# robertknight/ocrs

Hardware: AMD Instinct MI355X
Metric: pages/sec end-to-end (1024x1024) (higher is better)
Workload: dtype f32

## Files before the change

include/ocrs_amd.h:

```cpp
#ifndef OCRS_AMD_H
#define OCRS_AMD_H

#include <stddef.h>
#include <stdint.h>

#if defined(__GNUC__)
#define OCRS_API __attribute__((visibility("default")))
#else
#define OCRS_API
#endif

#ifdef __cplusplus
extern "C" {
#endif

typedef enum ocrs_status {
    OCRS_OK = 0,
    OCRS_ERR_INVALID_ARGUMENT = 1,
    OCRS_ERR_MODEL_NOT_LOADED = 2,
    OCRS_ERR_MODEL_DIMS = 3,
    OCRS_ERR_RUN_FAILED = 4,
    OCRS_ERR_WRONG_OUTPUT = 5,
    OCRS_ERR_IMAGE_SOURCE = 6,
    OCRS_ERR_DEVICE = 7,
    OCRS_ERR_IO = 8,
    OCRS_ERR_CAPACITY = 9
} ocrs_status;

OCRS_API const char* ocrs_last_error(void);

#define OCRS_ABI_VERSION 6u
OCRS_API uint32_t ocrs_abi_version(void);

OCRS_API void ocrs_buffer_free(void* p);

OCRS_API ocrs_status ocrs_device_count(int* n);
OCRS_API ocrs_status ocrs_set_device(int device);
OCRS_API ocrs_status ocrs_get_device(int* device);

OCRS_API ocrs_status ocrs_ctc_beam_search(const float* logp, int t, int c, uint32_t width, int impl, uint32_t** labels,
                                          uint32_t** positions, size_t* n);
OCRS_API ocrs_status ocrs_ctc_beam_search_scored(const float* logp, int t, int c, uint32_t width, int impl, uint32_t** labels,
                                                 uint32_t** positions, size_t* n, double* score, float** step_logp);

OCRS_API ocrs_status ocrs_gru_tile_plan(const int32_t* lengths_desc, size_t n_lines, int hidden, int32_t* n_clusters, int32_t* waves,
                                        int16_t* tiles);

OCRS_API ocrs_status ocrs_coalescer_selftest(int n_threads, int requests_per_thread, int max_active, int max_pages,
                                             long window_us, int fail_every, uint64_t out[5]);

OCRS_API ocrs_status ocrs_set_option(const char* name, long value);
OCRS_API ocrs_status ocrs_option_name(int index, const char** name);

OCRS_API ocrs_status ocrs_device_pool_stats(int device, uint64_t out[12]);
OCRS_API ocrs_status ocrs_device_pool_configure(int device, uint64_t device_cached_cap_bytes, uint64_t pinned_cached_cap_bytes);
OCRS_API ocrs_status ocrs_device_pool_trim(int device);

typedef enum { OCRS_ISOLATION_AUTO = 0, OCRS_ISOLATION_NONE = 1 } ocrs_isolation;
OCRS_API ocrs_status ocrs_device_set_isolation(int device, ocrs_isolation policy);
OCRS_API ocrs_status ocrs_device_isolation(int device, int out[3]);

typedef struct ocrs_model ocrs_model;

OCRS_API ocrs_status ocrs_model_load_file(const char* path, ocrs_model** out);
OCRS_API ocrs_status ocrs_model_load_bytes(const void* data, size_t len, ocrs_model** out);
OCRS_API ocrs_status ocrs_model_load_file_on_device(const char* path, int device, ocrs_model** out);
OCRS_API ocrs_status ocrs_model_load_bytes_on_device(const void* data, size_t len, int device, ocrs_model** out);
OCRS_API ocrs_status ocrs_model_device(const ocrs_model* m, int* device);

typedef int (*ocrs_model_run_fn)(void* user, const float* input, const int64_t in_shape[4], float** output,
                                 int64_t out_shape[4], int* out_ndim);
OCRS_API ocrs_status ocrs_model_from_callback(const int64_t input_shape[4],
                                     ocrs_model_run_fn run, void* user, ocrs_model** out);

OCRS_API ocrs_status ocrs_model_input_shape(const ocrs_model* m, int64_t dims[4], uint8_t is_fixed[4]);

typedef struct ocrs_run_options {
    int timing;
} ocrs_run_options;

OCRS_API ocrs_status ocrs_model_run(const ocrs_model* m, const float* input, const int64_t in_shape[4],
                           const ocrs_run_options* opts, float** output, int64_t out_shape[4], int* out_ndim);

OCRS_API ocrs_status ocrs_model_flops(const ocrs_model* m, const int64_t in_shape[4], double* flops);

OCRS_API void ocrs_model_free(ocrs_model* m);

typedef struct ocrs_engine ocrs_engine;
typedef struct ocrs_page ocrs_page;

typedef enum ocrs_numerics { OCRS_NUMERICS_EXACT = 0, OCRS_NUMERICS_RELAXED = 1, OCRS_NUMERICS_REDUCED = 2 } ocrs_numerics;

typedef enum ocrs_decode_method {
    OCRS_DECODE_GREEDY = 0,
    OCRS_DECODE_BEAM_SEARCH = 1
} ocrs_decode_method;

typedef struct ocrs_engine_params {
    const ocrs_model* detection_model;
    const ocrs_model* recognition_model;
    int debug;
    ocrs_decode_method decode_method;
    uint32_t beam_width;
    const char* alphabet;
    const char* allowed_chars;
    ocrs_numerics numerics;
    int coalesce;
    int coalesce_pages;
    int coalesce_window_us;
    int layout_threads;
    int64_t rec_max_pixels;
} ocrs_engine_params;

OCRS_API ocrs_status ocrs_engine_new(const ocrs_engine_params* params, ocrs_engine** out);
OCRS_API void ocrs_engine_free(ocrs_engine* e);
OCRS_API ocrs_status ocrs_engine_device(const ocrs_engine* e, int* device);
OCRS_API ocrs_status ocrs_engine_set_option(ocrs_engine* e, const char* name, long value);
OCRS_API ocrs_status ocrs_engine_get_option(const ocrs_engine* e, const char* name, long* value);

typedef enum ocrs_dim_order { OCRS_HWC = 0, OCRS_CHW = 1 } ocrs_dim_order;
typedef enum ocrs_pixel_type { OCRS_U8 = 0, OCRS_F32 = 1 } ocrs_pixel_type;

OCRS_API ocrs_status ocrs_image_source_check_bytes(size_t len, uint32_t width, uint32_t height, uint32_t* channels);

OCRS_API ocrs_status ocrs_engine_prepare_input(const ocrs_engine* e, const void* pixels, ocrs_pixel_type type,
                                      ocrs_dim_order order, int height, int width, int channels,
                                      ocrs_page** out);
OCRS_API ocrs_status ocrs_engine_prepare_input_batch(const ocrs_engine* e, const void* const* pixels, size_t n,
                                                     ocrs_pixel_type type, ocrs_dim_order order, int height, int width,
                                                     int channels, ocrs_page** out);
OCRS_API ocrs_status ocrs_engine_prepare_input_device(const ocrs_engine* e, const void* d_pixels, ocrs_pixel_type type,
                                             ocrs_dim_order order, int height, int width, int channels,
// ... 272 lines not shown
```

ocrs_amd/_lib.py:

```python
import ctypes as C
import os

_HERE = os.path.dirname(os.path.abspath(__file__))
LIB_PATH = os.environ.get("OCRS_AMD_LIB") or os.path.join(_HERE, "libocrs_amd.so")

OCRS_OK = 0
STATUS_NAMES = {
    0: "OK", 1: "INVALID_ARGUMENT", 2: "MODEL_NOT_LOADED", 3: "MODEL_DIMS", 4: "RUN_FAILED", 5: "WRONG_OUTPUT",
    6: "IMAGE_SOURCE", 7: "DEVICE", 8: "IO", 9: "CAPACITY",
}

RUN_FN = C.CFUNCTYPE(C.c_int, C.c_void_p, C.POINTER(C.c_float), C.POINTER(C.c_int64), C.POINTER(C.POINTER(C.c_float)),
                     C.POINTER(C.c_int64), C.POINTER(C.c_int))


class EngineParams(C.Structure):
    _fields_ = [("detection_model", C.c_void_p), ("recognition_model", C.c_void_p), ("debug", C.c_int),
                ("decode_method", C.c_int), ("beam_width", C.c_uint32), ("alphabet", C.c_char_p),
                ("allowed_chars", C.c_char_p), ("numerics", C.c_int), ("coalesce", C.c_int), ("coalesce_pages", C.c_int),
                ("coalesce_window_us", C.c_int), ("layout_threads", C.c_int), ("rec_max_pixels", C.c_int64)]


class GroupParams(C.Structure):
    _fields_ = [("detection_model", C.c_void_p), ("detection_model_len", C.c_size_t), ("recognition_model", C.c_void_p),
                ("recognition_model_len", C.c_size_t), ("devices", C.POINTER(C.c_int)), ("n_devices", C.c_size_t),
                ("debug", C.c_int), ("decode_method", C.c_int), ("beam_width", C.c_uint32), ("alphabet", C.c_char_p),
                ("allowed_chars", C.c_char_p), ("gather", C.c_int), ("numerics", C.c_int), ("coalesce", C.c_int),
                ("coalesce_pages", C.c_int), ("coalesce_window_us", C.c_int), ("layout_threads", C.c_int), ("rec_max_pixels", C.c_int64),
                ("min_block", C.c_int), ("shared_block", C.c_int)]


class RunOptions(C.Structure):
    _fields_ = [("timing", C.c_int)]


class TextCharC(C.Structure):
    _fields_ = [("ch", C.c_uint32), ("top", C.c_int32), ("left", C.c_int32), ("bottom", C.c_int32),
                ("right", C.c_int32)]


class OcrsError(RuntimeError):
    def __init__(self, status, message):
        super().__init__(message)
        self.status = status
        self.status_name = STATUS_NAMES.get(status, str(status))


DECLARED_SYMBOLS = [
    "ocrs_last_error", "ocrs_buffer_free", "ocrs_device_count", "ocrs_set_device", "ocrs_set_option", "ocrs_ctc_beam_search", "ocrs_model_load_file",
    "ocrs_model_load_bytes", "ocrs_model_from_callback", "ocrs_model_input_shape", "ocrs_model_run",
    "ocrs_model_flops", "ocrs_model_free", "ocrs_engine_new", "ocrs_engine_free", "ocrs_image_source_check_bytes",
    "ocrs_engine_prepare_input", "ocrs_engine_prepare_input_device", "ocrs_page_free", "ocrs_page_dims",
    "ocrs_page_image", "ocrs_engine_detect_words", "ocrs_engine_detect_words_batch",
    "ocrs_engine_detect_text_pixels", "ocrs_engine_detection_threshold", "ocrs_engine_find_text_lines",
    "ocrs_engine_find_text_lines_batch",
    "ocrs_engine_recognize_text", "ocrs_engine_recognize_text_batch", "ocrs_engine_recognize_tokens",
    "ocrs_engine_prepare_recognition_input", "ocrs_text_item_rotated_rect", "ocrs_rotated_rect_corners", "ocrs_engine_get_text", "ocrs_device_malloc", "ocrs_device_free",
    "ocrs_device_upload", "ocrs_device_synchronize", "ocrs_device_measure_peaks", "ocrs_engine_enable_timing", "ocrs_stage_count",
    "ocrs_stage_name", "ocrs_engine_stage_times", "ocrs_kernel_class_count", "ocrs_kernel_class_name",
    "ocrs_engine_kernel_stats", "ocrs_engine_set_kernel_timing_mask", "ocrs_gru_tile_plan", "ocrs_host_malloc", "ocrs_host_free", "ocrs_engine_prepare_input_batch",
    "ocrs_get_device", "ocrs_model_load_file_on_device", "ocrs_model_load_bytes_on_device", "ocrs_model_device", "ocrs_engine_device",
    "ocrs_engine_group_new", "ocrs_engine_group_free", "ocrs_engine_group_size", "ocrs_engine_group_member", "ocrs_group_deal",
    "ocrs_group_prepare_input_batch", "ocrs_group_prepare_input_device_batch", "ocrs_group_detect_words_batch",
    "ocrs_group_recognize_text_batch", "ocrs_group_gather", "ocrs_group_final_gather", "ocrs_group_worker_threads", "ocrs_group_last_gather", "ocrs_device_malloc_on", "ocrs_engine_coalesce_stats", "ocrs_coalescer_selftest", "ocrs_engine_kernel_mfma_flops", "ocrs_engine_prepare_input_jpeg", "ocrs_jpeg_decode_rgb", "ocrs_jpeg_info", "ocrs_jpeg_coefficients",
    "ocrs_group_member_stats", "ocrs_numa_parse_cpulist", "ocrs_numa_bind_selftest", "ocrs_engine_recognize_logits", "ocrs_engine_set_option", "ocrs_engine_get_option", "ocrs_option_name", "ocrs_device_pool_stats", "ocrs_device_pool_configure", "ocrs_device_pool_trim",
    "ocrs_device_set_isolation", "ocrs_device_isolation", "ocrs_group_set_replay", "ocrs_abi_version",
    "ocrs_engine_recognize_text_scored", "ocrs_engine_recognize_text_batch_scored", "ocrs_ctc_beam_search_scored",
    "ocrs_engine_run_recognition_ops",
    "ocrs_engine_detect_words_scored", "ocrs_engine_detect_words_batch_scored", "ocrs_group_detect_words_batch_scored",
    "ocrs_engine_find_text_lines_indexed", "ocrs_engine_find_text_lines_batch_indexed",
    "ocrs_detection_tile_plan", "ocrs_engine_detect_words_tiled", "ocrs_engine_detect_words_batch_tiled",
    "ocrs_engine_detect_text_pixels_tiled", "ocrs_group_detect_words_batch_tiled",
    "ocrs_line_frame", "ocrs_line_char_boxes", "ocrs_engine_prepare_recognition_input_rectified",
    "ocrs_engine_recognize_text_rectified", "ocrs_engine_recognize_text_batch_rectified",
    "ocrs_group_recognize_text_batch_rectified", "ocrs_engine_recognize_tokens_rectified",
    "ocrs_engine_rotate_page", "ocrs_engine_rotate_pages", "ocrs_unrotate_rects", "ocrs_unrotate_chars",
    "ocrs_orientation_vote", "ocrs_engine_detect_orientation", "ocrs_engine_page_from_grey",
    "ocrs_engine_resize_page", "ocrs_engine_resize_pages", "ocrs_work_size", "ocrs_rescale_rects",
    "ocrs_engine_detect_words_at", "ocrs_engine_detect_words_batch_at",
    "ocrs_normalize_params_default", "ocrs_normalize_params_check", "ocrs_engine_normalize_page", "ocrs_engine_normalize_pages",
    "ocrs_skew_params_default", "ocrs_skew_params_check", "ocrs_skew_table", "ocrs_engine_skew_scores", "ocrs_engine_estimate_skew",
    "ocrs_engine_warp_page", "ocrs_engine_warp_pages", "ocrs_deskew_map", "ocrs_unwarp_rects", "ocrs_unwarp_chars",
]

ABI_VERSION = 6
TILE_OVERLAP_DEFAULT = 100
RESAMPLE_FILTERS = {"auto": 0, "bilinear": 1, "area": 2}
POLARITIES = {"auto": 0, "keep": 1, "invert": 2}


class NormalizeParams(C.Structure):
    _fields_ = [("tile", C.c_int32), ("polarity", C.c_int32), ("flatten", C.c_int32), ("levels", C.c_int32)]


class NormalizeInfo(C.Structure):
    _fields_ = [("dark", C.c_int32), ("white", C.c_int32), ("lo", C.c_int32), ("hi", C.c_int32), ("vote", C.c_int64),
                ("counted", C.c_uint64)]

    def as_dict(self):
        return {"dark": int(self.dark), "vote": int(self.vote), "white": int(self.white), "lo": int(self.lo), "hi": int(self.hi),
                "counted": int(self.counted)}


class SkewParams(C.Structure):
    _fields_ = [("max_deg", C.c_double), ("coarse_step_deg", C.c_double), ("fine_step_deg", C.c_double), ("work_max_side", C.c_int32),
                ("reserved", C.c_int32)]


class SkewInfo(C.Structure):
    _fields_ = [("angle_deg", C.c_double), ("best_score", C.c_uint64), ("second_score", C.c_uint64), ("fine_score", C.c_uint64),
                ("work_h", C.c_int32), ("work_w", C.c_int32), ("coarse_index", C.c_int32), ("fine_index", C.c_int32)]


_lib = None


def lib():
    global _lib
    if _lib is None:
        if not os.path.exists(LIB_PATH):
            raise OcrsError(7, "libocrs_amd.so is not built: run `python -m ocrs_amd.build` "
                               "(there is no CPU fallback for the HIP engine)")
        L = C.CDLL(LIB_PATH)
        L.ocrs_abi_version.restype = C.c_uint32
        if L.ocrs_abi_version() != ABI_VERSION:
            raise OcrsError(7, "libocrs_amd.so has ABI version %d, this binding was written for %d: rebuild (python -m ocrs_amd.build)"
                            % (L.ocrs_abi_version(), ABI_VERSION))
        L.ocrs_last_error.restype = C.c_char_p
        L.ocrs_engine_detection_threshold.restype = C.c_float
        L.ocrs_engine_detection_threshold.argtypes = [C.c_void_p]
        L.ocrs_stage_name.restype = C.c_char_p
        L.ocrs_kernel_class_name.restype = C.c_char_p
        L.ocrs_buffer_free.argtypes = [C.c_void_p]
        for name in ("ocrs_model_free", "ocrs_engine_free", "ocrs_page_free", "ocrs_engine_group_free"):
            getattr(L, name).argtypes = [C.c_void_p]
            getattr(L, name).restype = None
        _lib = L
    return _lib


def check(status):
    if status != OCRS_OK:
        msg = lib().ocrs_last_error()
        raise OcrsError(status, msg.decode("utf-8", "replace") if msg else STATUS_NAMES.get(status, "error"))


def device_count():
# ... 122 lines not shown
```

ocrs_amd/csrc/abi.cpp:

```cpp
#include <cstdio>
#include <fstream>
#include <thread>

#include <atomic>
#include "abi_util.hpp"
#include "coalesce_selftest.hpp"
#include "engine.hpp"
#include "host_pool.hpp"
#include "jpeg.hpp"
#include "kernels.hpp"
#include "page_ops.hpp"

using namespace ocrs;
using namespace ocrs::geom;

using namespace ocrs::abi;

extern "C" {

const char* ocrs_last_error(void) { return last_error().c_str(); }

void ocrs_buffer_free(void* p) { free(p); }

ocrs_status ocrs_device_count(int* n) {
    return guarded([&] {
        int c = 0;
        hipError_t e = hipGetDeviceCount(&c);
        if (e != hipSuccess) c = 0;
        *n = c;
    });
}

ocrs_status ocrs_set_device(int device) {
    return guarded([&] { select_device(device); });
}

ocrs_status ocrs_get_device(int* device) {
    return guarded([&] {
        if (!device) fail(OCRS_ERR_INVALID_ARGUMENT, "null argument");
        *device = default_device();
    });
}

ocrs_status ocrs_gru_tile_plan(const int32_t* lengths_desc, size_t n_lines, int hidden, int32_t* n_clusters, int32_t* waves,
                               int16_t* tiles) {
    return guarded([&] {
        if (!lengths_desc || !n_clusters || !waves || !tiles || n_lines == 0 || n_lines > (size_t)1 << 20)
            fail(OCRS_ERR_INVALID_ARGUMENT, "bad argument");
        for (size_t i = 0; i < n_lines; i++)
            if (lengths_desc[i] < 1 || (i > 0 && lengths_desc[i] > lengths_desc[i - 1]))
                fail(OCRS_ERR_INVALID_ARGUMENT, "lengths must be positive and descending");
        int ncl = 0;
        if (!k::gru_tile_plan(lengths_desc, (int)n_lines, hidden, &ncl, waves, tiles))
            fail(OCRS_ERR_CAPACITY, "no persistent-kernel plan for this shape (the engine then runs the recurrence as one fused launch per time step)");
        *n_clusters = ncl;
    });
}

ocrs_status ocrs_coalescer_selftest(int n_threads, int requests_per_thread, int max_active, int max_pages, long window_us,
                                    int fail_every, uint64_t out[5]) {
    return guarded([&] {
        if (!out || n_threads < 1 || requests_per_thread < 1 || max_pages < 1) fail(OCRS_ERR_INVALID_ARGUMENT, "bad argument");
        coalescer_selftest(n_threads, requests_per_thread, max_active, max_pages, window_us, fail_every, out);
    });
}

namespace {

void beam_search_hook(const float* logp, int t, int c, uint32_t width, int impl, std::vector<uint32_t>* l,
                      std::vector<uint32_t>* p, double* score, std::vector<float>* step_logp) {
    if (impl == 2 && t > 0) {
        DeviceScope bind(-1);
        if (!k::ctc_beam_supported(c, (int)width)) fail(OCRS_ERR_CAPACITY, "beam search on the GPU supports up to 128 classes and width 128");
        Workspace ws;
        std::vector<int32_t> meta(1 + t + 1);
        meta[0] = t;
        for (int i = 0; i <= t; i++) meta[1 + i] = i;
        int32_t* d_meta = ws.alloc_n<int32_t>(meta.size());
        float* d_logp = ws.alloc_n<float>((size_t)t * c);
        ws.upload(d_meta, meta.data(), meta.size() * sizeof(int32_t));
        ws.upload(d_logp, logp, (size_t)t * c * sizeof(float));
        const size_t arena = k::ctc_beam_arena_entries(t, (int)width);
        int2* d_nodes = ws.alloc_n<int2>(arena);
        int2* d_posn = ws.alloc_n<int2>(arena);
        uint32_t* d_ol = ws.alloc_n<uint32_t>(t);
        uint32_t* d_op = ws.alloc_n<uint32_t>(t);
        int32_t* d_cnt = ws.alloc_n<int32_t>(1);
        double* d_score = score ? ws.alloc_n<double>(1) : nullptr;
        float* d_slp = score ? ws.alloc_n<float>(t) : nullptr;
        k::ctc_beam_packed(d_logp, d_meta, d_meta + 1, 1, t, c, (int)width, nullptr, d_nodes, d_posn, d_ol, d_op, d_cnt, ws.s(),
                           d_score, d_slp);
        std::vector<uint32_t> hl(t), hp(t);
        std::vector<float> hs(score ? t : 0);
        int32_t cnt = 0;
        ws.download(hl.data(), d_ol, (size_t)t * 4);
        ws.download(hp.data(), d_op, (size_t)t * 4);
        ws.download(&cnt, d_cnt, 4);
        if (score) {
            ws.download(score, d_score, sizeof(double));
            ws.download(hs.data(), d_slp, (size_t)t * sizeof(float));
        }
        ws.sync();
        OCRS_HIP(hipGetLastError());
        l->assign(hl.begin(), hl.begin() + cnt);
        p->assign(hp.begin(), hp.begin() + cnt);
        if (score) step_logp->assign(hs.begin(), hs.begin() + cnt);
    } else {
        double bs = 0.0;
        const std::vector<CtcStep> st = t == 0 ? std::vector<CtcStep>()
                                              : (impl == 1 ? ctc_beam_search_reference(logp, t, c, c, width, &bs)
                                                           : ctc_beam_search(logp, t, c, c, width, &bs));
        l->resize(st.size()); p->resize(st.size());
        for (size_t i = 0; i < st.size(); i++) { (*l)[i] = st[i].label; (*p)[i] = st[i].pos; }
        if (score) score_line(logp, t, c, c, nullptr, st, &bs, step_logp, score);
    }
}

}

ocrs_status ocrs_ctc_beam_search(const float* logp, int t, int c, uint32_t width, int impl, uint32_t** labels,
                                 uint32_t** positions, size_t* n) {
    return guarded([&] {
        if (!logp || !labels || !positions || !n || t < 0 || c < 1) fail(OCRS_ERR_INVALID_ARGUMENT, "bad argument");
        std::vector<uint32_t> l, p;
        beam_search_hook(logp, t, c, width, impl, &l, &p, nullptr, nullptr);
        *labels = dup_buffer(l);
        *positions = dup_buffer(p);
        *n = l.size();
    });
}

ocrs_status ocrs_ctc_beam_search_scored(const float* logp, int t, int c, uint32_t width, int impl, uint32_t** labels,
                                        uint32_t** positions, size_t* n, double* score, float** step_logp) {
    return guarded([&] {
        if (!logp || !labels || !positions || !n || !score || !step_logp || t < 0 || c < 1)
            fail(OCRS_ERR_INVALID_ARGUMENT, "bad argument");
        std::vector<uint32_t> l, p;
        std::vector<float> s;
        double sc = 0.0;
        beam_search_hook(logp, t, c, width, impl, &l, &p, &sc, &s);
        *labels = dup_buffer(l);
        *positions = dup_buffer(p);
        *step_logp = dup_buffer(s);
        *n = l.size();
        *score = sc;
    });
}

uint32_t ocrs_abi_version(void) { return OCRS_ABI_VERSION; }

static void check_option_set(int r, const char* name, long value) {
    if (r == 1) fail(OCRS_ERR_INVALID_ARGUMENT, "unknown option '%s'", name ? name : "(null)");
    if (r == 2) fail(OCRS_ERR_INVALID_ARGUMENT, "option '%s': value %ld is out of range", name, value);
}

ocrs_status ocrs_set_option(const char* name, long value) {
    return guarded([&] { check_option_set(set_option(name, value), name, value); });
}

ocrs_status ocrs_engine_set_option(ocrs_engine* e, const char* name, long value) {
    return guarded([&] {
        if (!e) fail(OCRS_ERR_INVALID_ARGUMENT, "null argument");
        check_option_set(set_option(e->tuning, name, value), name, value);
    });
}

ocrs_status ocrs_engine_get_option(const ocrs_engine* e, const char* name, long* value) {
    return guarded([&] {
        if (!e || !value) fail(OCRS_ERR_INVALID_ARGUMENT, "null argument");
        if (!get_option(e->tuning, name, value)) fail(OCRS_ERR_INVALID_ARGUMENT, "unknown option '%s'", name ? name : "(null)");
    });
}

ocrs_status ocrs_option_name(int index, const char** name) {
    return guarded([&] {
        if (!name) fail(OCRS_ERR_INVALID_ARGUMENT, "null argument");
        *name = option_name(index);
    });
}

ocrs_status ocrs_device_pool_stats(int device, uint64_t out[12]) {
    return guarded([&] {
        if (!out) fail(OCRS_ERR_INVALID_ARGUMENT, "null argument");
        DeviceContext& c = device_context(device < 0 ? default_device() : device);
        const PoolStats d = c.pool.stats(), h = c.host_pool.stats();
        const uint64_t v[12] = {d.live, d.cached, d.cap, d.peak_live, d.driver_allocs, d.driver_frees,
                                h.live, h.cached, h.cap, h.peak_live, h.driver_allocs, h.driver_frees};
        for (int i = 0; i < 12; i++) out[i] = v[i];
    });
}

ocrs_status ocrs_device_pool_trim(int device) {
    return guarded([&] {
        DeviceContext& c = device_context(device < 0 ? default_device() : device);
        DeviceScope bind(c.device);
        {
            std::lock_guard<std::mutex> heavy(c.heavy_phase);
            OCRS_HIP(hipStreamSynchronize(c.heavy_stream()));
            c.heavy_arena.clear();
        }
        c.pool.trim();
    });
}

ocrs_status ocrs_device_set_isolation(int device, ocrs_isolation policy) {
    return guarded([&] {
        if (policy != OCRS_ISOLATION_AUTO && policy != OCRS_ISOLATION_NONE) fail(OCRS_ERR_INVALID_ARGUMENT, "unknown isolation policy %d", (int)policy);
        DeviceContext& c = device_context(device < 0 ? default_device() : device);
        DeviceScope bind(c.device);
        c.set_isolation(policy == OCRS_ISOLATION_NONE ? DeviceContext::ISO_NONE : DeviceContext::ISO_AUTO);
    });
}

ocrs_status ocrs_device_isolation(int device, int out[3]) {
    return guarded([&] {
        if (!out) fail(OCRS_ERR_INVALID_ARGUMENT, "null argument");
        DeviceContext& c = device_context(device < 0 ? default_device() : device);
        DeviceScope bind(c.device);
        out[0] = (int)c.current_mode();
        out[1] = c.relaxed_engine_count();
        out[2] = c.cu_count();
    });
}

ocrs_status ocrs_device_pool_configure(int device, uint64_t device_cached_cap_bytes, uint64_t pinned_cached_cap_bytes) {
    return guarded([&] {
        DeviceContext& c = device_context(device < 0 ? default_device() : device);
        if (device_cached_cap_bytes) c.pool.set_cap(device_cached_cap_bytes);
        if (pinned_cached_cap_bytes) c.host_pool.set_cap(pinned_cached_cap_bytes);
    });
}

ocrs_status ocrs_model_load_bytes_on_device(const void* data, size_t len, int device, ocrs_model** out) {
    return guarded([&] {
        if (!data || !out) fail(OCRS_ERR_INVALID_ARGUMENT, "null argument");
        auto m = std::make_unique<ocrs_model>();
// ... 81 lines not shown
        std::vector<float> host((size_t)os.count());
        ws.download(host.data(), d_out, host.size() * sizeof(float));
        ws.sync();
        if (os.seq) {
            out_shape[0] = os.n; out_shape[1] = os.h; out_shape[2] = os.c; out_shape[3] = 1;
            *out_ndim = 3;
        } else {
            if (os.c != 1) {
                std::vector<float> t(host.size());
                for (int64_t b = 0; b < os.n; b++)
                    for (int64_t y = 0; y < os.h; y++)
                        for (int64_t x = 0; x < os.w; x++)
                            for (int64_t ch = 0; ch < os.c; ch++)
                                t[((b * os.c + ch) * os.h + y) * os.w + x] = host[((b * os.h + y) * os.w + x) * os.c + ch];
                host.swap(t);
            }
            out_shape[0] = os.n; out_shape[1] = os.c; out_shape[2] = os.h; out_shape[3] = os.w;
            *out_ndim = 4;
        }
        *output = dup_buffer(host);
    });
}

ocrs_status ocrs_model_flops(const ocrs_model* m, const int64_t in_shape[4], double* flops) {
    return guarded([&] {
        if (!m || !in_shape || !flops) fail(OCRS_ERR_INVALID_ARGUMENT, "null argument");
        if (m->impl->is_callback()) { *flops = 0; return; }
        *flops = static_cast<const HipModel*>(m->impl.get())->flops((int)in_shape[0], (int)in_shape[2], (int)in_shape[3]);
    });
}

void ocrs_model_free(ocrs_model* m) { delete m; }

ocrs_status ocrs_engine_new(const ocrs_engine_params* params, ocrs_engine** out) {
    return guarded([&] {
        if (!params || !out) fail(OCRS_ERR_INVALID_ARGUMENT, "null argument");
        *out = make_engine(*params).release();
    });
}

ocrs_status ocrs_engine_device(const ocrs_engine* e, int* device) {
    return guarded([&] {
        if (!e || !device) fail(OCRS_ERR_INVALID_ARGUMENT, "null argument");
        *device = e->device;
    });
}

void ocrs_engine_free(ocrs_engine* e) { delete e; }

ocrs_status ocrs_image_source_check_bytes(size_t len, uint32_t width, uint32_t height, uint32_t* channels) {
    return guarded([&] {
        const size_t channel_len = (size_t)width * height;
        if (channel_len == 0) fail(OCRS_ERR_IMAGE_SOURCE, "channel count is not 1, 3 or 4");
        if (len % channel_len != 0) fail(OCRS_ERR_IMAGE_SOURCE, "data length is not a multiple of `width * height`");
        const size_t ch = len / channel_len;
        if (!(ch == 1 || ch == 3 || ch == 4)) fail(OCRS_ERR_IMAGE_SOURCE, "channel count is not 1, 3 or 4");
        if (channels) *channels = (uint32_t)ch;
    });
}

ocrs_status ocrs_engine_prepare_input(const ocrs_engine* e, const void* pixels, ocrs_pixel_type type,
                                      ocrs_dim_order order, int height, int width, int channels, ocrs_page** out) {
    return guarded_engine(e, [&] {
        if (!e || !out) fail(OCRS_ERR_INVALID_ARGUMENT, "null argument");
        check_image_args(pixels, height, width, channels);
        Workspace ws;
        const size_t bytes = (size_t)height * width * channels * (type == OCRS_U8 ? 1 : 4);
        void* d_px = ws.alloc(bytes);
        OCRS_HIP(hipMemcpyAsync(d_px, pixels, bytes, hipMemcpyHostToDevice, ws.s()));
        ocrs_page* p = make_page(d_px, type, order, height, width, channels, ws.s(), e->tm());
        ws.sync();
        if (e->tm()) e->tm()->collect();
        *out = p;
    });
}

ocrs_status ocrs_engine_prepare_input_batch(const ocrs_engine* e, const void* const* pixels, size_t n, ocrs_pixel_type type,
                                            ocrs_dim_order order, int height, int width, int channels, ocrs_page** out) {
    return guarded_engine(e, [&] {
        if (!e || !out || (n > 0 && !pixels)) fail(OCRS_ERR_INVALID_ARGUMENT, "null argument");
        for (size_t i = 0; i < n; i++) check_image_args(pixels[i], height, width, channels);
        Workspace ws;
        const size_t bytes = (size_t)height * width * channels * (type == OCRS_U8 ? 1 : 4);
        std::vector<std::unique_ptr<ocrs_page>> made;
        for (size_t i = 0; i < n; i++) {
            void* d_px = ws.alloc(bytes);
            OCRS_HIP(hipMemcpyAsync(d_px, pixels[i], bytes, hipMemcpyHostToDevice, ws.s()));
            made.emplace_back(make_page(d_px, type, order, height, width, channels, ws.s(), e->tm()));
        }
        ws.sync();
        if (e->tm()) e->tm()->collect();
        for (size_t i = 0; i < n; i++) out[i] = made[i].release();
    });
}

ocrs_status ocrs_engine_prepare_input_device(const ocrs_engine* e, const void* d_pixels, ocrs_pixel_type type,
                                             ocrs_dim_order order, int height, int width, int channels,
                                             ocrs_page** out) {
    return guarded_engine(e, [&] {
        if (!e || !out) fail(OCRS_ERR_INVALID_ARGUMENT, "null argument");
        check_image_args(d_pixels, height, width, channels);
        Workspace ws;
        ocrs_page* p = make_page(d_pixels, type, order, height, width, channels, ws.s(), e->tm());
        ws.sync();
        if (e->tm()) e->tm()->collect();
        *out = p;
    });
}

namespace {
uint8_t* jpeg_to_device_rgb(Workspace& ws, const void* jpeg, size_t len, int* height, int* width, size_t* coef_bytes) {
    const ocrs::jpeg::Coefficients c = ocrs::jpeg::decode_coefficients(static_cast<const uint8_t*>(jpeg), len);
    const size_t nb = c.nblocks();
    uint64_t* d_mask = ws.alloc_n<uint64_t>(nb);
    uint32_t* d_off = ws.alloc_n<uint32_t>(nb + 1);
    int16_t* d_val = ws.alloc_n<int16_t>(c.values.size() + 1);
    uint16_t* d_q = ws.alloc_n<uint16_t>(4 * 64);
    ws.upload(d_mask, c.mask.data(), nb * sizeof(uint64_t));
    ws.upload(d_off, c.offset.data(), (nb + 1) * sizeof(uint32_t));
    ws.upload(d_val, c.values.data(), c.values.size() * sizeof(int16_t));
    ws.upload(d_q, c.quant, sizeof c.quant);
    uint8_t* d_samples = ws.alloc_n<uint8_t>(k::jpeg_sample_bytes(c));
    uint8_t* d_rgb = ws.alloc_n<uint8_t>((size_t)c.width * c.height * 3);
    k::jpeg_decode(c, d_mask, d_off, d_val, d_q, d_samples, d_rgb, ws.s());
    OCRS_HIP(hipGetLastError());
    *height = c.height;
    *width = c.width;
    if (coef_bytes) *coef_bytes = nb * 12 + 4 + c.values.size() * 2 + sizeof c.quant;
    return d_rgb;
}
}

ocrs_status ocrs_engine_prepare_input_jpeg(const ocrs_engine* e, const void* jpeg, size_t len, ocrs_page** out, size_t* coef_bytes) {
    return guarded_engine(e, [&] {
        if (!e || !jpeg || !out) fail(OCRS_ERR_INVALID_ARGUMENT, "null argument");
        Workspace ws;
        int h = 0, w = 0;
        const uint8_t* d_rgb = jpeg_to_device_rgb(ws, jpeg, len, &h, &w, coef_bytes);
        ocrs_page* p = make_page(d_rgb, OCRS_U8, OCRS_HWC, h, w, 3, ws.s(), e->tm());
        ws.sync();
        if (e->tm()) e->tm()->collect();
        *out = p;
    });
}

ocrs_status ocrs_jpeg_decode_rgb(int device, const void* jpeg, size_t len, uint8_t** rgb, int* height, int* width, size_t* coef_bytes) {
    return guarded_on(device, [&] {
        if (!jpeg || !rgb || !height || !width) fail(OCRS_ERR_INVALID_ARGUMENT, "null argument");
        Workspace ws;
        const uint8_t* d_rgb = jpeg_to_device_rgb(ws, jpeg, len, height, width, coef_bytes);
        std::vector<uint8_t> host((size_t)*height * *width * 3);
        ws.download(host.data(), d_rgb, host.size());
        ws.sync();
        *rgb = dup_buffer(host);
    });
}

ocrs_status ocrs_jpeg_info(const void* jpeg, size_t len, int* height, int* width, int* components, int* progressive, size_t* nonzero) {
    return guarded([&] {
        if (!jpeg) fail(OCRS_ERR_INVALID_ARGUMENT, "null argument");
        const ocrs::jpeg::Coefficients c = ocrs::jpeg::decode_coefficients(static_cast<const uint8_t*>(jpeg), len);
        if (height) *height = c.height;
        if (width) *width = c.width;
        if (components) *components = c.ncomp;
        if (progressive) *progressive = c.progressive ? 1 : 0;
        if (nonzero) *nonzero = c.values.size();
    });
}

ocrs_status ocrs_jpeg_coefficients(const void* jpeg, size_t len, int32_t geom[28], uint16_t quant[256], int16_t** coef, size_t* n_blocks) {
    return guarded([&] {
        if (!jpeg || !geom || !quant || !coef || !n_blocks) fail(OCRS_ERR_INVALID_ARGUMENT, "null argument");
// ... 601 lines not shown
```

ocrs_amd/csrc/abi_util.cpp:

```cpp
#include "abi_util.hpp"

#include "kernels.hpp"
#include "page_ops.hpp"

namespace ocrs {
namespace abi {

using namespace ocrs::geom;

void check_pages_on(const ocrs_engine* e, const ocrs_page* const* pages, size_t n) {
    for (size_t i = 0; i < n; i++) {
        if (!pages[i]) fail(OCRS_ERR_INVALID_ARGUMENT, "null page");
        if (pages[i]->device() != e->device)
            fail(OCRS_ERR_INVALID_ARGUMENT, "page %zu lives on device %d, the engine on device %d", i, pages[i]->device(),
                 e->device);
    }
}

std::u32string decode_utf8(const char* s) {
    std::u32string out;
    const unsigned char* p = reinterpret_cast<const unsigned char*>(s);
    while (*p) {
        uint32_t c = *p++;
        int extra = c >= 0xF0 ? 3 : c >= 0xE0 ? 2 : c >= 0xC0 ? 1 : 0;
        if (extra) c &= (0x3F >> extra);
        while (extra-- > 0 && *p) c = (c << 6) | (*p++ & 0x3F);
        out.push_back((char32_t)c);
    }
    return out;
}

void append_utf8(std::string& s, uint32_t c) {
    if (c < 0x80) s.push_back((char)c);
    else if (c < 0x800) { s.push_back((char)(0xC0 | (c >> 6))); s.push_back((char)(0x80 | (c & 0x3F))); }
    else if (c < 0x10000) {
        s.push_back((char)(0xE0 | (c >> 12))); s.push_back((char)(0x80 | ((c >> 6) & 0x3F)));
        s.push_back((char)(0x80 | (c & 0x3F)));
    } else {
        s.push_back((char)(0xF0 | (c >> 18))); s.push_back((char)(0x80 | ((c >> 12) & 0x3F)));
        s.push_back((char)(0x80 | ((c >> 6) & 0x3F))); s.push_back((char)(0x80 | (c & 0x3F)));
    }
}

static const char kDefaultAlphabet[] =
    " 0123456789!\"#$%&'()*+,-./:;<=>?@[\\]^_`{|}~\xE2\x82\xAC"
    "ABCDEFGHIJKLMNOPQRSTUVWXYZabcdefghijklmnopqrstuvwxyz";

std::vector<std::vector<RotatedRect>> unpack_lines(const float* rects, const size_t* offsets, size_t first, size_t last) {
    std::vector<std::vector<RotatedRect>> lines;
    for (size_t i = first; i < last; i++) lines.push_back(unpack_words(rects + 6 * offsets[i], offsets[i + 1] - offsets[i]));
    return lines;
}

ocrs_page* make_page(const void* d_pixels, ocrs_pixel_type type, ocrs_dim_order order, int height, int width, int channels,
                     hipStream_t st, StageTimers* T) {
    auto page = new_page(height, width);
    {
        StageScope sc(T, ST_PREPARE, st);
        k::prepare_image(d_pixels, type == OCRS_U8, order == OCRS_HWC, height, width, channels, page->grey.as<float>(), st);
    }
    OCRS_HIP(hipGetLastError());
    return page.release();
}

void check_image_args(const void* pixels, int height, int width, int channels) {
    if (!pixels) fail(OCRS_ERR_INVALID_ARGUMENT, "pixels is null");
    if (!(channels == 1 || channels == 3 || channels == 4)) fail(OCRS_ERR_IMAGE_SOURCE, "channel count is not 1, 3 or 4");
    if (height <= 0 || width <= 0) fail(OCRS_ERR_INVALID_ARGUMENT, "image has no pixels");
}

std::unique_ptr<ocrs_engine> make_engine(const ocrs_engine_params& params) {
    auto e = std::make_unique<ocrs_engine>();
    e->detection = params.detection_model ? params.detection_model->impl.get() : nullptr;
    e->recognition = params.recognition_model ? params.recognition_model->impl.get() : nullptr;
    const int dd = e->detection ? e->detection->device : -1, rd = e->recognition ? e->recognition->device : -1;
    if (dd >= 0 && rd >= 0 && dd != rd)
        fail(OCRS_ERR_INVALID_ARGUMENT, "detection model is on device %d, recognition model on device %d", dd, rd);
    e->device = dd >= 0 ? dd : rd >= 0 ? rd : default_device();
    e->debug = params.debug != 0;
    e->tuning = default_tuning();
    if (params.numerics != OCRS_NUMERICS_EXACT && params.numerics != OCRS_NUMERICS_RELAXED && params.numerics != OCRS_NUMERICS_REDUCED)
        fail(OCRS_ERR_INVALID_ARGUMENT, "unknown numerics mode %d", (int)params.numerics);
    e->tuning.v[OPT_NUMERICS] = (long)params.numerics;
    if (params.numerics != OCRS_NUMERICS_EXACT) e->count_relaxed(device_context(e->device));
    if (params.coalesce) e->tuning.v[OPT_COALESCE] = params.coalesce < 0 ? 0 : params.coalesce;
    if (params.coalesce_pages) e->tuning.v[OPT_COALESCE_PAGES] = params.coalesce_pages < 0 ? 1 : params.coalesce_pages;
    if (params.coalesce_window_us) e->tuning.v[OPT_COALESCE_WINDOW_US] = params.coalesce_window_us < 0 ? 0 : params.coalesce_window_us;
    if (params.layout_threads > 0) e->tuning.v[OPT_LAYOUT_THREADS] = params.layout_threads;
    if (params.rec_max_pixels > 0) e->tuning.v[OPT_REC_MAX_PIXELS] = (long)params.rec_max_pixels;
    e->decode_method = params.decode_method;
    e->beam_width = params.beam_width ? params.beam_width : 100;
    e->alphabet = decode_utf8(params.alphabet ? params.alphabet : kDefaultAlphabet);
    if (params.allowed_chars) {
        const std::u32string allowed = decode_utf8(params.allowed_chars);
        e->excluded.assign(e->alphabet.size() + 1, 0);
        for (size_t i = 0; i < e->alphabet.size(); i++)
            if (allowed.find(e->alphabet[i]) == std::u32string::npos) e->excluded[i + 1] = 1;
        e->has_excluded = true;
        DeviceScope bind(e->device);
        e->d_excluded = DevBuf(e->excluded.size());
        OCRS_HIP(hipMemcpy(e->d_excluded.p, e->excluded.data(), e->excluded.size(), hipMemcpyHostToDevice));
    }
    e->init_coalescers();
    return e;
}

void flatten_chars(const ocrs_engine* e, const std::vector<RecResult>& res, std::vector<ocrs_text_char>* flat, std::vector<size_t>* offs) {
    flat->clear();
    offs->assign(1, 0);
    for (const RecResult& r : res) {
        for (const TextChar& c : e->text_line_from_result(r))
            flat->push_back(ocrs_text_char{c.ch, c.rect.top, c.rect.left, c.rect.bottom, c.rect.right});
        offs->push_back(flat->size());
    }
}

}
}
```

ocrs_amd/csrc/abi_util.hpp:

```cpp
#pragma once
#include <cstdlib>
#include <cstring>
#include <memory>
#include <string>
#include <vector>

#include "engine.hpp"

namespace ocrs {
namespace abi {

template <class F>
ocrs_status guarded(F&& f) {
    try {
        f();
        set_last_error("");
        return OCRS_OK;
    } catch (const Error& e) {
        set_last_error(e.what());
        return e.status;
    } catch (const std::bad_alloc&) {
        set_last_error("out of host memory");
        return OCRS_ERR_DEVICE;
    } catch (const std::exception& e) {
        set_last_error(e.what());
        return OCRS_ERR_RUN_FAILED;
    }
}

template <class F>
ocrs_status guarded_on(int device, F&& f) {
    return guarded([&] {
        DeviceScope bind(device);
        f();
    });
}

template <class F>
ocrs_status guarded_engine(const ocrs_engine* e, F&& f) {
    return guarded([&] {
        DeviceScope bind(e ? e->device : -1);
        TuningScope tune(e ? &e->tuning : nullptr);
        f();
    });
}

template <class T>
T* dup_buffer(const std::vector<T>& v) {
    T* p = static_cast<T*>(malloc(std::max<size_t>(v.size(), 1) * sizeof(T)));
    if (!p) throw std::bad_alloc();
    if (!v.empty()) memcpy(p, v.data(), v.size() * sizeof(T));
    return p;
}

inline void append_rects(std::vector<float>& flat, const std::vector<geom::RotatedRect>& rects) {
    for (const geom::RotatedRect& r : rects) {
        float a[6];
        r.to_array(a);
        flat.insert(flat.end(), a, a + 6);
    }
}

inline std::vector<geom::RotatedRect> unpack_words(const float* rects6, size_t n) {
    std::vector<geom::RotatedRect> words(n);
    for (size_t i = 0; i < n; i++) words[i] = geom::RotatedRect::from_array(rects6 + 6 * i);
    return words;
}

template <class PerPage>
void pack_words(const std::vector<std::vector<geom::RotatedRect>>& rr, const DetScores* sc, float** rects, size_t* offsets,
                float** score, uint32_t** pixels, PerPage&& per_page) {
    std::vector<float> flat, fscore;
    std::vector<uint32_t> fpixels;
    offsets[0] = 0;
    for (size_t i = 0; i < rr.size(); i++) {
        const size_t first = flat.size();
        append_rects(flat, rr[i]);
        per_page(i, flat.data() + first, rr[i].size());
        if (sc) {
            fscore.insert(fscore.end(), sc->score[i].begin(), sc->score[i].end());
            fpixels.insert(fpixels.end(), sc->pixels[i].begin(), sc->pixels[i].end());
        }
        offsets[i + 1] = flat.size() / 6;
    }
    if (sc) {
        *score = dup_buffer(fscore);
        *pixels = dup_buffer(fpixels);
    }
    *rects = dup_buffer(flat);
}
inline void pack_words(const std::vector<std::vector<geom::RotatedRect>>& rr, const DetScores* sc, float** rects, size_t* offsets,
                       float** score, uint32_t** pixels) {
    pack_words(rr, sc, rects, offsets, score, pixels, [](size_t, float*, size_t) {});
}

inline int tile_overlap_arg(int overlap) { return overlap < 0 ? OCRS_TILE_OVERLAP_DEFAULT : overlap; }

void check_pages_on(const ocrs_engine* e, const ocrs_page* const* pages, size_t n);
std::u32string decode_utf8(const char* s);
void append_utf8(std::string& s, uint32_t c);
std::vector<std::vector<geom::RotatedRect>> unpack_lines(const float* rects, const size_t* offsets, size_t first, size_t last);
ocrs_page* make_page(const void* d_pixels, ocrs_pixel_type type, ocrs_dim_order order, int height, int width, int channels,
                     hipStream_t st, StageTimers* T);
void check_image_args(const void* pixels, int height, int width, int channels);
std::unique_ptr<ocrs_engine> make_engine(const ocrs_engine_params& params);
void flatten_chars(const ocrs_engine* e, const std::vector<RecResult>& res, std::vector<ocrs_text_char>* flat, std::vector<size_t>* offs);

}
}
```

ocrs_amd/csrc/common.cpp:

```cpp
#include "common.hpp"

#include <chrono>
#include <climits>
#include <cstdint>
#include <cstdlib>
#include <cstring>

#include <algorithm>
#include <atomic>
#include <condition_variable>
#include <deque>
#include <system_error>

namespace ocrs {

static thread_local std::string g_last_error;

void set_last_error(const std::string& msg) { g_last_error = msg; }
const std::string& last_error() { return g_last_error; }

namespace {
std::atomic<int> g_default_device{0};
thread_local DeviceContext* t_ctx = nullptr;
constexpr int kMaxDevices = 64;
std::mutex g_ctx_mu;
std::atomic<DeviceContext*> g_ctx[kMaxDevices];
}

DeviceContext& device_context(int device) {
    if (device < 0 || device >= kMaxDevices) fail(OCRS_ERR_INVALID_ARGUMENT, "device index %d out of range", device);
    DeviceContext* c = g_ctx[device].load(std::memory_order_acquire);
    if (c) return *c;
    std::lock_guard<std::mutex> g(g_ctx_mu);
    c = g_ctx[device].load(std::memory_order_relaxed);
    if (!c) {
        c = new DeviceContext(device);
        g_ctx[device].store(c, std::memory_order_release);
    }
    return *c;
}

int default_device() { return g_default_device.load(); }

void select_device(int device) {
    int n = 0;
    OCRS_HIP(hipGetDeviceCount(&n));
    if (device < 0 || device >= n) fail(OCRS_ERR_INVALID_ARGUMENT, "device %d does not exist (%d visible)", device, n);
    OCRS_HIP(hipSetDevice(device));
    g_default_device.store(device);
}

DeviceContext& ctx() {
    if (t_ctx) return *t_ctx;
    return device_context(default_device());
}

DeviceScope::DeviceScope(int device) : prev_(t_ctx) {
    DeviceContext& c = device_context(device < 0 ? default_device() : device);
    if (!prev_ && hipGetDevice(&restore_) != hipSuccess) {
        (void)hipGetLastError();
        restore_ = -1;
    }
    const hipError_t e = hipSetDevice(c.device);
    if (e != hipSuccess) {
        (void)hipGetLastError();
        fail(OCRS_ERR_DEVICE, "cannot bind to HIP device %d: %s", c.device, hipGetErrorString(e));
    }
    t_ctx = &c;
}

DeviceScope::~DeviceScope() {
    const int here = t_ctx ? t_ctx->device : -1;
    t_ctx = prev_;
    const int back = prev_ ? prev_->device : restore_;
    if (back >= 0 && back != here && hipSetDevice(back) != hipSuccess) (void)hipGetLastError();
}

const char* const kStageNames[ST_COUNT] = {
    "prepare_image", "resize_to_model", "detection_cnn", "resize_threshold", "ccl",      "contour_rects",
    "line_crop",     "rec_conv",        "rec_gru",       "rec_head",         "ctc_decode"};

const char* const kKernelClassNames[KC_COUNT] = {
    "gemm_conv3x3_mfma", "gemm_pointwise_mfma", "gemm_convt_mfma", "gemm_gru_input_mfma", "gemm_gru_hidden_mfma",
    "gemm_linear_mfma",  "dwconv3x3",           "conv_direct",     "pool",                "padcat",
    "conv1x1_sigmoid",   "gru_gates",           "logsoftmax_argmax", "other",
    "det_fused_block",   "det_stream_wave_block", "det_stream_rows_block"};

static size_t round_size(size_t n) {
    if (n <= (1u << 20)) return (n + 255) & ~size_t(255);
    size_t p = size_t(1) << 20;
    while (p * 2 <= n) p *= 2;
    size_t step = p / 8;
    return ((n + step - 1) / step) * step;
}

namespace {
struct Trimmer;
Trimmer& trimmer();
struct Trimmer {
    struct Item { int device; void* p; std::atomic<uint64_t>* freed; };
    std::mutex mu;
    std::condition_variable cv;
    std::deque<Item> q;
    bool started = false;
    std::atomic<bool> exiting{false};
    std::mutex freeing;
    void run() {
        for (;;) {
            Item it;
            {
                std::unique_lock<std::mutex> lk(mu);
                cv.wait(lk, [&] { return !q.empty(); });
                it = q.front();
                q.pop_front();
            }
            std::lock_guard<std::mutex> f(freeing);
            if (exiting.load()) continue;
            bool ok;
            if (it.device >= 0) ok = hipSetDevice(it.device) == hipSuccess && hipFree(it.p) == hipSuccess;
            else ok = hipHostFree(it.p) == hipSuccess;
            (void)hipGetLastError();
            if (ok && it.freed) it.freed->fetch_add(1, std::memory_order_relaxed);
// ... 109 lines not shown
        cached_ += it->second;
        live_bytes_ -= it->second;
        live_.erase(it);
        const uint64_t cap = cap_locked();
        while (cached_ > cap && !free_.empty()) {
            auto big = std::prev(free_.end());
            drop.push_back(big->second);
            cached_ -= big->first;
            free_.erase(big);
        }
    }
    for (void* q : drop) trimmer().give(device_, q, &frees_);
}

void DevicePool::trim() {
    std::lock_guard<std::mutex> g(mu_);
    for (auto& kv : free_) { (void)hipFree(kv.second); frees_++; }
    free_.clear();
    cached_ = 0;
}

DevicePool::~DevicePool() {
}

void* HostPool::alloc(size_t bytes) {
    const size_t sz = round_size(bytes);
    {
        std::lock_guard<std::mutex> g(mu_);
        auto it = free_.lower_bound(sz);
        if (it != free_.end() && it->first <= sz + sz / 4) {
            void* p = it->second;
            const size_t got = it->first;
            free_.erase(it);
            cached_ -= got;
            live_[p] = got;
            live_bytes_ += got;
            peak_live_ = std::max(peak_live_, live_bytes_);
            return p;
        }
    }
    void* p = nullptr;
    OCRS_HIP(hipHostMalloc(&p, sz, hipHostMallocPortable));
    std::lock_guard<std::mutex> g(mu_);
    live_[p] = sz;
    live_bytes_ += sz;
    peak_live_ = std::max(peak_live_, live_bytes_);
    allocs_++;
    return p;
}

void HostPool::release(void* p) {
    if (!p) return;
    std::vector<void*> drop;
    {
        std::lock_guard<std::mutex> g(mu_);
        auto it = live_.find(p);
        if (it == live_.end()) return;
        free_.emplace(it->second, p);
        cached_ += it->second;
        live_bytes_ -= it->second;
        live_.erase(it);
        while (cached_ > cap_ && !free_.empty()) {
            auto big = std::prev(free_.end());
            drop.push_back(big->second);
            cached_ -= big->first;
            free_.erase(big);
        }
    }
    for (void* q : drop) trimmer().give(-1, q, &frees_);
}

void HostPool::set_cap(uint64_t bytes) {
    std::lock_guard<std::mutex> g(mu_);
    cap_ = bytes;
}

PoolStats HostPool::stats() {
    std::lock_guard<std::mutex> g(mu_);
    PoolStats st;
    st.live = live_bytes_; st.cached = cached_; st.cap = cap_; st.peak_live = peak_live_; st.driver_allocs = allocs_; st.driver_frees = frees_;
    return st;
}

hipStream_t DeviceContext::heavy_stream() {
    std::lock_guard<std::mutex> g(lazy_mu_);
    if (!heavy_) {
        DeviceScope bind(device);
        int least = 0, greatest = 0;
        OCRS_HIP(hipDeviceGetStreamPriorityRange(&least, &greatest));
        OCRS_HIP(hipStreamCreateWithPriority(&heavy_, hipStreamNonBlocking, greatest));
    }
    return heavy_;
}

hipStream_t DeviceContext::recurrent_stream(int mode) {
    if (mode == MODE_SERIAL) return heavy_stream();
    std::lock_guard<std::mutex> g(lazy_mu_);
    if (!recurrent_) {
        DeviceScope bind(device);
        int least = 0, greatest = 0;
        OCRS_HIP(hipDeviceGetStreamPriorityRange(&least, &greatest));
        OCRS_HIP(hipStreamCreateWithPriority(&recurrent_, hipStreamNonBlocking, greatest));
    }
    return recurrent_;
}

static thread_local int t_lease_depth[kMaxDevices] = {0};

template <class F> void DeviceContext::switch_isolation(F&& change) {
    if (t_lease_depth[device] > 0) fail(OCRS_ERR_INVALID_ARGUMENT, "the isolation regime of device %d cannot change from inside one of its requests", device);
    std::unique_lock<std::mutex> lk(iso_mu_);
    iso_cv_.wait(lk, [&] { return !switching_; });
    const Mode before = mode_locked();
    switching_ = true;
    struct Done { DeviceContext* c; ~Done() { c->switching_ = false; c->iso_cv_.notify_all(); } } done{this};
    const Isolation p0 = policy_;
    const int r0 = relaxed_;
    change();
    if (mode_locked() == before) return;
    const Isolation p1 = policy_;
    const int r1 = relaxed_;
    policy_ = p0; relaxed_ = r0;
    iso_cv_.wait(lk, [&] { return leases_ == 0; });
    {
        DeviceScope bind(device);
        if (hipDeviceSynchronize() != hipSuccess) (void)hipGetLastError();
    }
    policy_ = p1; relaxed_ = r1;
}

DeviceContext::Mode DeviceContext::lease_begin() {
    std::unique_lock<std::mutex> lk(iso_mu_);
    if (t_lease_depth[device] == 0) iso_cv_.wait(lk, [&] { return !switching_; });
    t_lease_depth[device]++;
    leases_++;
    return mode_locked();
}

void DeviceContext::lease_end() {
    std::lock_guard<std::mutex> lk(iso_mu_);
    t_lease_depth[device]--;
    if (--leases_ == 0) iso_cv_.notify_all();
}

void DeviceContext::add_relaxed_engine(int delta) {
    switch_isolation([&] { relaxed_ += delta; });
}

void DeviceContext::set_isolation(Isolation policy) {
    switch_isolation([&] { policy_ = policy; });
}

DeviceContext::Mode DeviceContext::current_mode() {
    std::lock_guard<std::mutex> lk(iso_mu_);
    return mode_locked();
}

int DeviceContext::relaxed_engine_count() {
    std::lock_guard<std::mutex> lk(iso_mu_);
    return relaxed_;
}

int DeviceContext::cu_count() {
    std::lock_guard<std::mutex> g(lazy_mu_);
    if (!cus_) {
        hipDeviceProp_t prop;
        OCRS_HIP(hipGetDeviceProperties(&prop, device));
        cus_ = prop.multiProcessorCount;
    }
    return cus_;
}

namespace {
struct OptDef { const char* name; const char* env; long def; };
const OptDef kOptDefs[OPT_COUNT] = {
    {"gru_mode", "OCRS_GRU_MODE", GRU_PERSISTENT},
    {"gru_gates", "OCRS_GRU_GATES", 1},
    {"gru_local", "OCRS_GRU_LOCAL", 1},
    {"det_fuse", "OCRS_DET_FUSE", 1},
    {"det_stream", "OCRS_DET_STREAM", 1},
    {"det_rows", "OCRS_DET_ROWS", 1},
    {"ccl_quad", "OCRS_CCL_QUAD", 1},
    {"conv12_fuse", "OCRS_CONV12_FUSE", 1},
    {"conv_flat", "OCRS_CONV_FLAT", 1},
    {"beam_gpu", "OCRS_BEAM_GPU", 1},
    {"det_tile_batch", "OCRS_DET_TILE_BATCH", 16},
    {"numerics", nullptr, 0},
    {"coalesce", nullptr, 2},
    {"coalesce_pages", nullptr, 16},
    {"coalesce_window_us", nullptr, 300},
    {"layout_threads", nullptr, 0},
    {"rec_max_pixels", nullptr, 0},
};
struct OptRange { long lo, hi; long also[4]; };
const OptRange kOptRanges[OPT_COUNT] = {
    {0, 1, {}}, {0, 1, {}}, {0, 1, {}}, {0, 2, {}}, {0, 1, {8, 14, 32}}, {0, 1, {8, 14, 20, 32}}, {0, 1, {}}, {0, 1, {}}, {0, 1, {}}, {0, 1, {}},
    {1, 1024, {}},
    {0, 2, {}}, {0, 64, {}}, {1, 4096, {}}, {0, 10000000, {}}, {0, 4096, {}}, {0, INT64_MAX, {}},
};
bool in_range(int i, long v) {
    const OptRange& r = kOptRanges[i];
    if (v >= r.lo && v <= r.hi) return true;
    for (long a : r.also) if (a && v == a) return true;
    return false;
}
const char* const kRetired[] = {"det_heavy", "det_tail", "gru_waves", "gru_background", "gru_scatter", "gru_gates_pack", "conv_occupancy",
                                "gx_heavy", "gemm_nfast", "conv_a_lds", "gru_heavy", "heavy_priority", "det_mfma"};
std::atomic<long> g_opts[OPT_COUNT];
std::once_flag g_opts_once;
void init_options() {
    for (int i = 0; i < OPT_COUNT; i++) {
        const char* e = kOptDefs[i].env ? getenv(kOptDefs[i].env) : nullptr;
        const long v = e && *e ? strtol(e, nullptr, 10) : kOptDefs[i].def;
        g_opts[i].store(in_range(i, v) ? v : kOptDefs[i].def);
    }
}
int find_option(const char* name, int count = OPT_PUBLIC_COUNT) {
    for (int i = 0; i < count; i++)
        if (name && i != OPT_NUMERICS && strcmp(name, kOptDefs[i].name) == 0) return i;
    return -1;
}
thread_local const Tuning* t_tuning = nullptr;
}

TuningScope::TuningScope(const Tuning* t) : prev_(t_tuning) { t_tuning = t; }
TuningScope::~TuningScope() { t_tuning = prev_; }
const Tuning* current_tuning() { return t_tuning; }

long option_long(Option o) {
    if (t_tuning) return __atomic_load_n(&t_tuning->v[o], __ATOMIC_RELAXED);
    std::call_once(g_opts_once, init_options);
    return g_opts[o].load(std::memory_order_relaxed);
}
int option(Option o) { return (int)option_long(o); }

Tuning default_tuning() {
    std::call_once(g_opts_once, init_options);
    Tuning t;
    for (int i = 0; i < OPT_COUNT; i++) t.v[i] = g_opts[i].load(std::memory_order_relaxed);
    return t;
}

const char* option_name(int i) { return i >= 0 && i < OPT_PUBLIC_COUNT ? kOptDefs[i].name : nullptr; }

int set_option(const char* name, long value) {
    std::call_once(g_opts_once, init_options);
    const int i = find_option(name);
    if (i < 0) {
        for (const char* r : kRetired) if (name && strcmp(name, r) == 0) return 0;
        return 1;
    }
    if (!in_range(i, value)) return 2;
    g_opts[i].store(value);
    return 0;
}

int set_option(Tuning& t, const char* name, long value) {
    const int i = find_option(name, OPT_COUNT);
    if (i < 0) return 1;
    if (!in_range(i, value)) return 2;
    __atomic_store_n(&t.v[i], value, __ATOMIC_RELAXED);
    return 0;
}

bool get_option(const Tuning& t, const char* name, long* value) {
    const int i = name && strcmp(name, "numerics") == 0 ? (int)OPT_NUMERICS : find_option(name, OPT_COUNT);
    if (i < 0) return false;
    *value = __atomic_load_n(&t.v[i], __ATOMIC_RELAXED);
    return true;
}

StreamLease::StreamLease(bool high_priority) : ctx_(&ctx()), high_(high_priority) {
    high_ = true;
    mode_ = ctx_->lease_begin();
    try {
        if (mode_ == DeviceContext::MODE_SERIAL) {
            s_ = ctx_->heavy_stream();
            shared_ = true;
            OCRS_HIP(hipEventCreateWithFlags(&done_, hipEventBlockingSync | hipEventDisableTiming));
            return;
        }
        {
            std::lock_guard<std::mutex> g(ctx_->stream_mu);
            auto& v = ctx_->streams;
            if (!v.empty()) {
                s_ = v.back().first;
                done_ = v.back().second;
                v.pop_back();
                return;
            }
        }
        int least = 0, greatest = 0;
        OCRS_HIP(hipDeviceGetStreamPriorityRange(&least, &greatest));
        OCRS_HIP(hipStreamCreateWithPriority(&s_, hipStreamNonBlocking, greatest));
        OCRS_HIP(hipEventCreateWithFlags(&done_, hipEventBlockingSync | hipEventDisableTiming));
    } catch (...) {
        ctx_->lease_end();
        throw;
    }
}

StreamLease::~StreamLease() {
    if (shared_) {
        (void)hipEventDestroy(done_);
    } else {
        std::lock_guard<std::mutex> g(ctx_->stream_mu);
        ctx_->streams.emplace_back(s_, done_);
    }
    ctx_->lease_end();
}

std::vector<StageTimers::Pending>& StageTimers::pending() {
    static thread_local std::vector<Pending> p;
    return p;
}
std::map<int, std::vector<hipEvent_t>>& StageTimers::thread_events() {
    static thread_local std::map<int, std::vector<hipEvent_t>> f;
    return f;
}
std::vector<hipEvent_t>& StageTimers::free_events() { return thread_events()[ctx().device]; }

hipEvent_t StageTimers::get_event() {
    auto& fe = free_events();
    if (!fe.empty()) {
        hipEvent_t e = fe.back();
        fe.pop_back();
        return e;
    }
    hipEvent_t e;
    OCRS_HIP(hipEventCreate(&e));
    return e;
}

int StageTimers::begin(int stage, hipStream_t s, uint64_t n_launches) {
    if (!enabled) return -1;
    Pending p{stage, get_event(), get_event(), n_launches, false, 0.0, 0.0, 0.0};
    OCRS_HIP(hipEventRecord(p.a, s));
    pending().push_back(p);
    return (int)pending().size() - 1;
}

int StageTimers::kbegin(int cls, hipStream_t s, double flops, double bytes, double mfma_flops) {
    if (!enabled || !kernels_enabled || !((kernel_mask >> cls) & 1u)) return -1;
    if (mfma_flops < 0.0) mfma_flops = cls <= KC_GEMM_LINEAR ? flops : 0.0;
    Pending p{cls, get_event(), get_event(), 1, true, flops, bytes, mfma_flops};
    OCRS_HIP(hipEventRecord(p.a, s));
    pending().push_back(p);
    return (int)pending().size() - 1;
}

void StageTimers::end(int token, hipStream_t s) {
    if (token < 0) return;
    auto& pd = pending();
    if ((size_t)token < pd.size()) (void)hipEventRecord(pd[token].b, s);
}

void StageTimers::collect() {
    auto& pd = pending();
    if (pd.empty()) return;
    double lms[ST_COUNT] = {0}, lkms[KC_COUNT] = {0}, lkf[KC_COUNT] = {0}, lkb[KC_COUNT] = {0}, lkm[KC_COUNT] = {0};
    uint64_t ln[ST_COUNT] = {0}, lkn[KC_COUNT] = {0};
    for (auto& p : pd) {
        float t = 0.f;
        if (hipEventSynchronize(p.b) == hipSuccess && hipEventElapsedTime(&t, p.a, p.b) == hipSuccess) {
            if (p.kernel) { lkms[p.stage] += t; lkn[p.stage] += 1; lkf[p.stage] += p.flops; lkb[p.stage] += p.bytes; lkm[p.stage] += p.mfma; }
            else { lms[p.stage] += t; ln[p.stage] += p.n; }
        }
        free_events().push_back(p.a);
        free_events().push_back(p.b);
    }
    pd.clear();
    std::lock_guard<std::mutex> g(mu);
    for (int i = 0; i < ST_COUNT; i++) { ms[i] += lms[i]; launches[i] += ln[i]; }
    for (int i = 0; i < KC_COUNT; i++) { kms[i] += lkms[i]; klaunches[i] += lkn[i]; kflops[i] += lkf[i]; kbytes[i] += lkb[i]; kmfma[i] += lkm[i]; }
}

void StageTimers::release_thread_events() {
    for (auto& p : pending()) { (void)hipEventDestroy(p.a); (void)hipEventDestroy(p.b); }
    pending().clear();
    for (auto& kv : thread_events()) {
        for (hipEvent_t e : kv.second) (void)hipEventDestroy(e);
        kv.second.clear();
    }
}

void StageTimers::reset() {
    std::lock_guard<std::mutex> g(mu);
    for (int i = 0; i < ST_COUNT; i++) { ms[i] = 0; launches[i] = 0; }
    for (int i = 0; i < KC_COUNT; i++) { kms[i] = 0; klaunches[i] = 0; kflops[i] = 0; kbytes[i] = 0; kmfma[i] = 0; }
}

// ... 2 lines not shown
```

ocrs_amd/csrc/common.hpp:

```cpp
#pragma once
#include <atomic>
#include <hip/hip_runtime.h>

#include <cstdarg>
#include <cstdint>
#include <cstdio>
#include <cstdlib>
#include <chrono>
#include <condition_variable>
#include <cstring>
#include <map>
#include <mutex>
#include <stdexcept>
#include <string>
#include <thread>
#include <vector>

#include "../../include/ocrs_amd.h"

namespace ocrs {

struct Error : std::runtime_error {
    ocrs_status status;
    Error(ocrs_status s, const std::string& msg) : std::runtime_error(msg), status(s) {}
};

[[noreturn]] inline void fail(ocrs_status s, const char* fmt, ...) {
    char buf[512];
    va_list ap;
    va_start(ap, fmt);
    vsnprintf(buf, sizeof buf, fmt, ap);
    va_end(ap);
    throw Error(s, buf);
}

#define OCRS_HIP(expr)                                                                              \
    do {                                                                                            \
        hipError_t _e = (expr);                                                                     \
        if (_e != hipSuccess)                                                                       \
            ::ocrs::fail(OCRS_ERR_DEVICE, "HIP error %s at %s:%d (%s)", hipGetErrorString(_e), __FILE__, \
                         __LINE__, #expr);                                                          \
    } while (0)

void set_last_error(const std::string& msg);


struct PoolStats { uint64_t live = 0, cached = 0, cap = 0, peak_live = 0, driver_allocs = 0, driver_frees = 0; };
class DevicePool {
  public:
    explicit DevicePool(int device) : device_(device) {}
    ~DevicePool();
    void* alloc(size_t bytes);
    void release(void* p);
    void trim();
    void set_cap(uint64_t bytes);
    PoolStats stats();
    int device() const { return device_; }

  private:
    uint64_t cap_locked();
    const int device_;
    std::mutex mu_;
    std::multimap<size_t, void*> free_;
    std::map<void*, size_t> live_;
    uint64_t cached_ = 0, live_bytes_ = 0, peak_live_ = 0, cap_ = 0, allocs_ = 0;
    std::atomic<uint64_t> frees_{0};
};

class HostPool {
  public:
    void* alloc(size_t bytes);
    void release(void* p);
    void set_cap(uint64_t bytes);
    PoolStats stats();

  private:
    std::mutex mu_;
    std::multimap<size_t, void*> free_;
    std::map<void*, size_t> live_;
    uint64_t cached_ = 0, live_bytes_ = 0, peak_live_ = 0, cap_ = uint64_t(1) << 30, allocs_ = 0;
    std::atomic<uint64_t> frees_{0};
};

struct DeviceContext {
    const int device;
    DevicePool pool;
    HostPool host_pool;
    std::mutex heavy_phase, rec_phase;
    hipStream_t heavy_stream();
    hipStream_t recurrent_stream(int mode = 0);
    enum Isolation { ISO_AUTO = 0, ISO_NONE = 1 };
    enum Mode { MODE_FREE = 0, MODE_SERIAL = 1 };
    Mode lease_begin();
    void lease_end();
    void add_relaxed_engine(int delta);
    void set_isolation(Isolation policy);
    Mode current_mode();
    int relaxed_engine_count();
    int cu_count();
    std::vector<struct DevBuf> heavy_arena;
    std::mutex stream_mu;
    std::vector<std::pair<hipStream_t, hipEvent_t>> streams;

    explicit DeviceContext(int d) : device(d), pool(d) {}

  private:
    Mode mode_locked() const { return policy_ == ISO_NONE || relaxed_ <= 0 ? MODE_FREE : MODE_SERIAL; }
    template <class F> void switch_isolation(F&& change);
    std::mutex lazy_mu_;
    hipStream_t heavy_ = nullptr, recurrent_ = nullptr;
    int cus_ = 0;
    std::mutex iso_mu_;
    std::condition_variable iso_cv_;
    int leases_ = 0, relaxed_ = 0;
    bool switching_ = false;
    Isolation policy_ = ISO_AUTO;
    friend class StreamLease;
};

DeviceContext& device_context(int device);
int default_device();
void select_device(int device);
DeviceContext& ctx();

class DeviceScope {
  public:
    explicit DeviceScope(int device);
    ~DeviceScope();
    DeviceScope(const DeviceScope&) = delete;
    DeviceScope& operator=(const DeviceScope&) = delete;

  private:
    DeviceContext* prev_;
    int restore_ = -1;
};

inline DevicePool& pool() { return ctx().pool; }
inline HostPool& host_pool() { return ctx().host_pool; }
inline hipStream_t heavy_stream() { return ctx().heavy_stream(); }

enum Option { OPT_GRU_MODE = 0, OPT_GRU_GATES, OPT_GRU_LOCAL, OPT_DET_FUSE, OPT_DET_STREAM, OPT_DET_ROWS, OPT_CCL_QUAD,
              OPT_CONV12_FUSE, OPT_CONV_FLAT, OPT_BEAM_GPU, OPT_DET_TILE_BATCH, OPT_PUBLIC_COUNT,
              OPT_NUMERICS = OPT_PUBLIC_COUNT,
              OPT_COALESCE, OPT_COALESCE_PAGES, OPT_COALESCE_WINDOW_US,
              OPT_LAYOUT_THREADS, OPT_REC_MAX_PIXELS,
              OPT_COUNT };
struct Tuning { long v[OPT_COUNT]; };
Tuning default_tuning();
int set_option(const char* name, long value);
int set_option(Tuning& t, const char* name, long value);
bool get_option(const Tuning& t, const char* name, long* value);
const char* option_name(int i);
class TuningScope {
  public:
    explicit TuningScope(const Tuning* t);
    ~TuningScope();
    TuningScope(const TuningScope&) = delete;
    TuningScope& operator=(const TuningScope&) = delete;
  private:
    const Tuning* prev_;
};
const Tuning* current_tuning();
enum { GRU_PERSISTENT = 0, GRU_STEP = 1 };
int option(Option o);

inline void allow_dynamic_lds(const void* kernel, std::atomic<uint64_t>& done) {
    int dev = 0;
    (void)hipGetDevice(&dev);
    const uint64_t bit = 1ull << (dev & 63);
    if (done.load(std::memory_order_relaxed) & bit) return;
    (void)hipFuncSetAttribute(kernel, hipFuncAttributeMaxDynamicSharedMemorySize, 160 * 1024);
    done.fetch_or(bit, std::memory_order_relaxed);
}
long option_long(Option o);
inline int gru_mode() { return option(OPT_GRU_MODE); }

struct DevBuf {
    void* p = nullptr;
    size_t bytes = 0;
    DevicePool* owner = nullptr;
    DevBuf() = default;
    explicit DevBuf(size_t n) : bytes(n), owner(n ? &pool() : nullptr) { p = n ? owner->alloc(n) : nullptr; }
    DevBuf(const DevBuf&) = delete;
    DevBuf& operator=(const DevBuf&) = delete;
    DevBuf(DevBuf&& o) noexcept : p(o.p), bytes(o.bytes), owner(o.owner) { o.p = nullptr; o.bytes = 0; o.owner = nullptr; }
    DevBuf& operator=(DevBuf&& o) noexcept {
        if (this != &o) { reset(); p = o.p; bytes = o.bytes; owner = o.owner; o.p = nullptr; o.bytes = 0; o.owner = nullptr; }
        return *this;
    }
    ~DevBuf() { reset(); }
    void reset() { if (p && owner) owner->release(p); p = nullptr; bytes = 0; owner = nullptr; }
    int device() const { return owner ? owner->device() : -1; }
    template <class T> T* as() const { return static_cast<T*>(p); }
};

struct PinnedBuf {
    void* p = nullptr;
    size_t bytes = 0;
    PinnedBuf() = default;
    explicit PinnedBuf(size_t n) : bytes(n) { if (n) OCRS_HIP(hipHostMalloc(&p, n, hipHostMallocPortable)); }
    PinnedBuf(const PinnedBuf&) = delete;
    PinnedBuf& operator=(const PinnedBuf&) = delete;
    ~PinnedBuf() { if (p) (void)hipHostFree(p); }
    template <class T> T* as() const { return static_cast<T*>(p); }
};

class StreamLease {
  public:
    explicit StreamLease(bool high_priority = false);
    ~StreamLease();
    hipStream_t get() const { return s_; }
    hipError_t wait_done() const noexcept {
        hipError_t e = hipEventRecord(done_, s_);
        if (e != hipSuccess) return e;
        for (int i = 0;; i++) {
            e = hipEventQuery(done_);
            if (e != hipErrorNotReady) return e;
            if (i < 64) std::this_thread::yield();
            else std::this_thread::sleep_for(std::chrono::microseconds(i < 256 ? 20 : 100));
        }
    }
    void sync() const { OCRS_HIP(wait_done()); }
    hipError_t sync_noexcept() const noexcept { return wait_done(); }
    DeviceContext::Mode mode() const { return mode_; }
    bool serial() const { return mode_ == DeviceContext::MODE_SERIAL; }
    hipStream_t conv_stream() const { return ctx_->heavy_stream(); }
    hipStream_t recurrent_stream() const { return ctx_->recurrent_stream((int)mode_); }

  private:
    DeviceContext* ctx_;
    DeviceContext::Mode mode_ = DeviceContext::MODE_FREE;
    bool shared_ = false;
    hipStream_t s_;
    hipEvent_t done_;
    bool high_;
};

enum Stage {
    ST_PREPARE = 0,
    ST_RESIZE_IN,
    ST_DET_CNN,
    ST_RESIZE_THRESH,
    ST_CCL,
    ST_CONTOUR_RECTS,
    ST_LINE_CROP,
    ST_REC_CONV,
    ST_REC_GRU,
    ST_REC_HEAD,
    ST_CTC,
    ST_COUNT
};
extern const char* const kStageNames[ST_COUNT];

enum KernelClass {
    KC_GEMM_CONV3X3 = 0, KC_GEMM_POINTWISE, KC_GEMM_CONVT, KC_GEMM_GRU_INPUT, KC_GEMM_GRU_HIDDEN, KC_GEMM_LINEAR,
    KC_DWCONV3X3, KC_CONV_DIRECT, KC_POOL, KC_PADCAT, KC_CONV1X1_SIGMOID, KC_GRU_GATES, KC_LOGSOFTMAX_ARGMAX,
    KC_OTHER, KC_DET_BLOCK, KC_DET_STREAM_WAVE, KC_DET_STREAM_ROWS, KC_COUNT
};
extern const char* const kKernelClassNames[KC_COUNT];

struct StageTimers {
    bool enabled = false;
    bool kernels_enabled = false;
    uint32_t kernel_mask = 0xffffffffu;
    std::mutex mu;
    double ms[ST_COUNT] = {0};
    uint64_t launches[ST_COUNT] = {0};
    double kms[KC_COUNT] = {0};
    uint64_t klaunches[KC_COUNT] = {0};
    double kflops[KC_COUNT] = {0};
    double kbytes[KC_COUNT] = {0};
    double kmfma[KC_COUNT] = {0};
    struct Pending { int stage; hipEvent_t a, b; uint64_t n; bool kernel; double flops, bytes, mfma; };
    static std::vector<Pending>& pending();
    int begin(int stage, hipStream_t s, uint64_t n_launches);
    int kbegin(int cls, hipStream_t s, double flops, double bytes, double mfma_flops = -1.0);
    void end(int token, hipStream_t s);
    void collect();
    void reset();
    static void release_thread_events();
  private:
    static std::vector<hipEvent_t>& free_events();
    static std::map<int, std::vector<hipEvent_t>>& thread_events();
    hipEvent_t get_event();
};

inline int ceil_div(int64_t a, int64_t b) { return (int)((a + b - 1) / b); }

struct StageScope {
    StageTimers* t; int token; hipStream_t s;
    StageScope(StageTimers* timers, int stage, hipStream_t stream, uint64_t n_launches = 1)
        : t(timers), token(timers ? timers->begin(stage, stream, n_launches) : -1), s(stream) {}
    ~StageScope() { if (t && token >= 0) t->end(token, s); }
};

struct Workspace {
    StreamLease stream;
    HostPool& hpool = host_pool();
    std::vector<DevBuf> bufs;
    std::vector<hipEvent_t> events;
    hipEvent_t make_event() {
        hipEvent_t e;
        OCRS_HIP(hipEventCreateWithFlags(&e, hipEventDisableTiming));
        events.push_back(e);
        return e;
    }
    Workspace() = default;
    explicit Workspace(bool high_priority) : stream(high_priority) {}
    std::vector<void*> upload_staging;
    void upload(void* d_dst, const void* h_src, size_t bytes) {
        if (!bytes) return;
        void* pin = hpool.alloc(bytes);
        memcpy(pin, h_src, bytes);
        upload_staging.push_back(pin);
        OCRS_HIP(hipMemcpyAsync(d_dst, pin, bytes, hipMemcpyHostToDevice, stream.get()));
    }
    struct Download { void* pinned; void* dst; size_t bytes; };
    std::vector<Download> downloads;
    void download(void* h_dst, const void* d_src, size_t bytes, hipStream_t st = nullptr) {
        if (!bytes) return;
        void* pin = hpool.alloc(bytes);
        downloads.push_back(Download{pin, h_dst, bytes});
        OCRS_HIP(hipMemcpyAsync(pin, d_src, bytes, hipMemcpyDeviceToHost, st ? st : stream.get()));
    }
    void download_2d(void* h_dst, const void* d_src, size_t d_pitch, size_t width, size_t rows, hipStream_t st = nullptr) {
        if (!width || !rows) return;
        void* pin = hpool.alloc(width * rows);
        downloads.push_back(Download{pin, h_dst, width * rows});
        OCRS_HIP(hipMemcpy2DAsync(pin, width, d_src, d_pitch, width, rows, hipMemcpyDeviceToHost, st ? st : stream.get()));
    }
    hipStream_t s() const { return stream.get(); }
    void* alloc(size_t bytes) { bufs.emplace_back(bytes ? bytes : 4); return bufs.back().p; }
    template <class T> T* alloc_n(size_t n) { return static_cast<T*>(alloc(n * sizeof(T))); }
    void finish_downloads(bool copy) {
        for (const Download& d : downloads) {
            if (copy) memcpy(d.dst, d.pinned, d.bytes);
            hpool.release(d.pinned);
        }
        downloads.clear();
        for (void* p : upload_staging) hpool.release(p);
        upload_staging.clear();
    }
    void sync() {
        stream.sync();
        finish_downloads(true);
    }
    ~Workspace() {
        (void)stream.sync_noexcept();
        finish_downloads(false);
        for (hipEvent_t e : events) (void)hipEventDestroy(e);
    }
};

const std::string& last_error();

}
```

ocrs_amd/csrc/engine.cpp:

```cpp
#include "engine.hpp"

#include <algorithm>
#include <limits>
#include <map>
#include <thread>

#include "kernels.hpp"

using namespace ocrs;
using namespace ocrs::geom;

TileAxisPlan ocrs::tile_axis_plan(int L, int M, int v) {
    if (L <= 0 || M <= 0 || v < 0 || v > M / 2) fail(OCRS_ERR_INVALID_ARGUMENT, "tile plan: length %d, model length %d, overlap %d", L, M, v);
    TileAxisPlan p;
    if (L <= M) {
        p.origin = {0};
        p.bound = {0, L};
        return p;
    }
    const int n = (L - v + (M - v) - 1) / (M - v);
    p.origin.resize(n);
    p.bound.resize(n + 1);
    for (int i = 0; i < n; i++) p.origin[i] = (int32_t)(((int64_t)i * (L - M)) / (n - 1));
    p.bound[0] = 0;
    p.bound[n] = L;
    for (int i = 1; i < n; i++) p.bound[i] = (p.origin[i - 1] + M + p.origin[i]) / 2;
    return p;
}

namespace {

struct SizeGroup {
    int h = 0, w = 0, first = 0, count = 0;
    int pad_bottom = 0, pad_right = 0, max_comp = 0;
    int64_t px = 0, arena = 0;
    uint8_t* d_mask = nullptr;
    float* d_map = nullptr;
    bool prepared = false;
    k::CclBuffers b{};
};
struct PageGroups {
    std::vector<SizeGroup> groups;
    std::vector<int> order;
    std::vector<int> pos_of;
    std::vector<int> group_of;
};

PageGroups group_pages_by_size(const ocrs_page* const* pages, size_t n) {
    PageGroups pg;
    std::vector<SizeGroup>& groups = pg.groups;
    pg.order.resize(n); pg.pos_of.resize(n); pg.group_of.resize(n);
    std::vector<int> gi(n);
    for (size_t i = 0; i < n; i++) {
        const int h = pages[i]->h, w = pages[i]->w;
        if (h <= 0 || w <= 0 || h > 65535 || w > 65535) fail(OCRS_ERR_INVALID_ARGUMENT, "unsupported page size %dx%d", h, w);
        size_t g = 0;
        while (g < groups.size() && (groups[g].h != h || groups[g].w != w)) g++;
        if (g == groups.size()) { groups.emplace_back(); groups[g].h = h; groups[g].w = w; }
        groups[g].count++;
        gi[i] = (int)g;
    }
    int at = 0;
    for (SizeGroup& g : groups) { g.first = at; at += g.count; g.count = 0; }
    for (size_t i = 0; i < n; i++) {
        SizeGroup& g = groups[gi[i]];
        pg.order[g.first + g.count] = (int)i;
        pg.pos_of[i] = g.first + g.count;
        pg.group_of[g.first + g.count] = gi[i];
        g.count++;
    }
    return pg;
}

const float* run_detector(const ocrs_engine& e, Workspace& ws, const float* d_in, int n, int in_h, int in_w, float* d_cb_out,
                          const int* run_order) {
    if (!e.detection->is_callback()) {
        TensorShape os;
        const float* d_prob =
            static_cast<const HipModel*>(e.detection)->run_device(ws, d_in, n, in_h, in_w, &os, e.tm(), nullptr, nullptr, true, e.debug);
        if (os.n != n || os.h != in_h || os.w != in_w || os.c != 1)
            fail(OCRS_ERR_WRONG_OUTPUT, "model output had unexpected type or shape: detection output [%d,%d,%d,%d]", os.n,
                 os.c, os.h, os.w);
        return d_prob;
    }
    const auto* cb = static_cast<const CallbackModel*>(e.detection);
// ... 1010 lines not shown
    int32_t* d_labels = w.alloc_n<int32_t>((size_t)plan.R);
    float* d_logp = nullptr;
    float* d_maxlp = (rq.scored && !beam) ? w.alloc_n<float>((size_t)plan.R) : nullptr;
    rq.hm->run_recognition_packed(w, pg, plan, (int)e.rec_input_height(), T, d_excl, d_labels, (beam || rq.want_logp) ? &d_logp : nullptr,
                                  d_maxlp);
    sub.gpu_beam = beam && option(OPT_BEAM_GPU) && k::ctc_beam_supported(C, (int)e.beam_width);
    if (rq.want_logp || (beam && !sub.gpu_beam)) {
        sub.logp.resize((size_t)plan.R * C);
        sub.off = plan.h_off;
        w.download(sub.logp.data(), d_logp, sub.logp.size() * sizeof(float), sst);
    }
    if (beam && !sub.gpu_beam) return;
    int2* d_nodes = nullptr;
    int2* d_posn = nullptr;
    if (sub.gpu_beam) {
        const size_t arena = k::ctc_beam_arena_entries(Tmax, (int)e.beam_width);
        d_nodes = w.alloc_n<int2>((size_t)M * arena);
        d_posn = w.alloc_n<int2>((size_t)M * arena);
    }
    uint32_t* d_ol = w.alloc_n<uint32_t>((size_t)M * Tmax);
    uint32_t* d_op = w.alloc_n<uint32_t>((size_t)M * Tmax);
    int32_t* d_cnt = w.alloc_n<int32_t>(M);
    float* d_slp = rq.scored ? w.alloc_n<float>((size_t)M * Tmax) : nullptr;
    double* d_score = rq.scored ? w.alloc_n<double>(M) : nullptr;
    {
        StageScope sc(T, ST_CTC, sst);
        if (sub.gpu_beam)
            k::ctc_beam_packed(d_logp, plan.d_Tm, plan.d_off, M, Tmax, C, (int)e.beam_width, d_excl, d_nodes, d_posn, d_ol, d_op, d_cnt,
                               sst, d_score, d_slp);
        else if (rq.scored)
            k::ctc_collapse_scored_packed(d_labels, d_maxlp, plan.d_Tm, plan.d_off, M, Tmax, d_ol, d_op, d_slp, d_cnt, d_score, sst);
        else
            k::ctc_collapse_packed(d_labels, plan.d_Tm, plan.d_off, M, Tmax, d_ol, d_op, d_cnt, sst);
    }
    download_steps(w, sst, (size_t)M, Tmax, d_ol, d_op, d_cnt, d_slp, d_score, &sub.dec);
}

void unpack_packed(const PackedRequest& rq, const Sub& sub) {
    const ocrs_engine& e = rq.e;
    const int C = rq.C;
    const size_t M = sub.slots.size();
    for (uint32_t st8 : sub.gru_status)
        if (st8) fail(OCRS_ERR_DEVICE, "GRU recurrence kernel timed out waiting for a peer workgroup (status 0x%x)", st8);
    auto row = [&](size_t m, int t) { return &sub.logp[((size_t)sub.off[t] + m) * C]; };
    if (rq.want_logp)
        for (size_t m = 0; m < M; m++) {
            auto& dst = rq.res[sub.slots[m].line].logp;
            dst.resize((size_t)sub.slots[m].T * C);
            for (int t = 0; t < sub.slots[m].T; t++) memcpy(&dst[(size_t)t * C], row(m, t), (size_t)C * sizeof(float));
        }
    if (e.decode_method == OCRS_DECODE_BEAM_SEARCH && !sub.gpu_beam) {
        const unsigned nth = (unsigned)std::max<size_t>(1, std::min<size_t>({(size_t)std::thread::hardware_concurrency(), (size_t)32, M}));
        std::vector<std::thread> th;
        for (unsigned w0 = 0; w0 < nth; w0++)
            th.emplace_back([&, w0] {
                std::vector<float> seq;
                for (size_t m = w0; m < M; m += nth)
                    beam_decode_line(e, sub.slots[m].T, C, [&](int t) { return row(m, t); }, seq, rq.scored, &rq.res[sub.slots[m].line]);
            });
        for (auto& t : th) t.join();
        return;
    }
    for (size_t m = 0; m < M; m++) take_steps(sub.dec, m, (uint32_t)sub.slots[m].T, &rq.res[sub.slots[m].line]);
}

void recognize_packed(const ocrs_engine& e, Workspace& ws, const std::vector<Chunk>& chunks, RecResult* res, bool scored, bool want_logp) {
    const auto* hm = static_cast<const HipModel*>(e.recognition);
    PackedRequest rq{e, hm, chunks, std::vector<int>(chunks.size()), 0, scored, want_logp, res};
    int ndim = hm->packed_split() < 0 ? 4 : 3;
    for (size_t c = 0; c < chunks.size() && ndim == 3; c++) {
        TensorShape os = hm->infer(1, (int)e.rec_input_height(), (int)chunks[c].gw);
        if (!os.seq) ndim = 4;
        rq.chunk_T[c] = os.n;
        rq.C = os.c;
    }
    check_rec_output(ndim, 0, 0, rq.C, e.alphabet.size());
    const int T_SPLIT = 160;
    size_t first_long = chunks.size();
    for (size_t c = 0; c < chunks.size(); c++)
        if (rq.chunk_T[c] > T_SPLIT) { first_long = c; break; }
    size_t n_long_lines = 0, n_short_lines = 0;
    for (size_t c = 0; c < chunks.size(); c++) (c >= first_long ? n_long_lines : n_short_lines) += chunks[c].members.size();
    const bool split = n_long_lines > 0 && n_short_lines >= 64;
    Workspace ws_long(true);
    Sub sub_long, sub_short;
    if (split) {
        {
            hipEvent_t crops = ws.make_event();
            OCRS_HIP(hipEventRecord(crops, ws.s()));
            OCRS_HIP(hipStreamWaitEvent(ws_long.s(), crops, 0));
        }
        launch_packed(rq, first_long, chunks.size(), ws_long, sub_long);
        launch_packed(rq, 0, first_long, ws, sub_short);
        ws_long.sync();
        ws.sync();
        unpack_packed(rq, sub_long);
        unpack_packed(rq, sub_short);
    } else {
        launch_packed(rq, 0, chunks.size(), ws, sub_short);
        ws.sync();
        unpack_packed(rq, sub_short);
    }
}

}

void ocrs_engine::recognize_lines(const ocrs_page* const* pages, size_t n_pages, RecResult* res, size_t L, bool scored,
                                  bool want_logp) const {
    if (L == 0) return;
    const uint32_t rec_h = rec_input_height();
    const bool callback = recognition->is_callback();

    std::map<uint32_t, std::vector<size_t>> groups;
    for (size_t i = 0; i < L; i++) groups[res[i].line.group_width].push_back(i);

    Workspace ws;
    std::vector<Chunk> chunks;
    std::vector<CropLine> crops;
    int64_t off = 0;
    for (auto& kv : groups) {
        const uint32_t gw = kv.first;
        if (gw == 0) continue;
        const size_t max_chunk = callback ? 20 : std::max<size_t>(1, 2457600 / gw);
        for (size_t c0 = 0; c0 < kv.second.size(); c0 += max_chunk) {
            Chunk ch;
            ch.gw = gw;
            ch.members.assign(kv.second.begin() + c0, kv.second.begin() + std::min(kv.second.size(), c0 + max_chunk));
            ch.off = off;
            for (size_t li : ch.members) {
                crops.push_back(CropLine{&res[li].line, gw, off});
                off += (int64_t)rec_h * gw;
            }
            chunks.push_back(std::move(ch));
        }
    }
    if ((double)off > std::max(rec_pixel_budget(), 2.0e9))
        fail(OCRS_ERR_CAPACITY, "text line too large for the recognition model (%lld input pixels)", (long long)off);
    float* d_all = stage_line_crops(ws, tm(), pages, n_pages, crops, (int)rec_h, off);
    if (!d_all) return;
    for (Chunk& ch : chunks) ch.ptr = d_all + ch.off;
    if (callback) {
        ws.sync();
        recognize_callback(*this, ws, chunks, res, scored);
    } else {
        recognize_packed(*this, ws, chunks, res, scored, want_logp);
    }
    if (StageTimers* T = tm()) T->collect();
}

std::vector<TextChar> ocrs_engine::text_line_from_result(const RecResult& res, std::vector<float>* char_logp) const {
    const RecLine& line = res.line;
    const uint32_t ctc_input_len = res.ctc_len;
    const std::vector<CtcStep>& steps = res.steps;
    std::vector<TextChar> out;
    if (char_logp) char_logp->clear();
    if (steps.empty() || ctc_input_len == 0) return out;
    if (line.rectified) {
        std::vector<uint32_t> pos(steps.size());
        for (size_t i = 0; i < steps.size(); i++) pos[i] = steps[i].pos;
        for (const auto& kv : rectified_char_boxes(line.frame, line.group_width, ctc_input_len, pos.data(), pos.size())) {
            const uint32_t idx = steps[kv.first].label - 1;
            out.push_back(TextChar{idx < alphabet.size() ? (uint32_t)alphabet[idx] : (uint32_t)'?', kv.second});
            if (char_logp) char_logp->push_back(res.step_logp[kv.first]);
        }
        return out;
    }
    const Rect line_rect = line.bounds;
    const float x_scale = (float)line_rect.width() / (float)line.resized_width;
    const uint32_t downsample = (uint32_t)rround((float)line.group_width / (float)ctc_input_len);
    for (size_t i = 0; i < steps.size(); i++) {
        const uint32_t start_x = steps[i].pos * downsample;
        const uint32_t end_x = i + 1 < steps.size() ? steps[i + 1].pos * downsample : line.resized_width;
        const int32_t sx = line_rect.left + as_i32((float)start_x * x_scale);
        const int32_t ex = line_rect.left + as_i32((float)end_x * x_scale);
        if (sx >= line_rect.right) continue;
        const uint32_t idx = steps[i].label - 1;
        const uint32_t ch = idx < alphabet.size() ? (uint32_t)alphabet[idx] : (uint32_t)'?';
        Rect r;
// ... 8 lines not shown
```

ocrs_amd/csrc/group.cpp:

```cpp
#include <dlfcn.h>
#include <rccl/rccl.h>

#include <atomic>

#include "abi_util.hpp"
#include "host_pool.hpp"
#include "numa.hpp"
#include "kernels.hpp"
#include "page_ops.hpp"

using namespace ocrs;
using namespace ocrs::abi;
using namespace ocrs::geom;

namespace {

struct RcclApi {
    void* handle = nullptr;
    std::string path, error;
    bool accepts_duplicate_devices = false;
    decltype(&ncclCommInitAll) CommInitAll = nullptr;
    decltype(&ncclCommDestroy) CommDestroy = nullptr;
    decltype(&ncclGroupStart) GroupStart = nullptr;
    decltype(&ncclGroupEnd) GroupEnd = nullptr;
// ... 437 lines not shown
        *out = g.release();
    });
}

void ocrs_engine_group_free(ocrs_engine_group* g) { delete g; }

ocrs_status ocrs_engine_group_size(const ocrs_engine_group* g, size_t* n) {
    return guarded([&] {
        if (!g || !n) fail(OCRS_ERR_INVALID_ARGUMENT, "null argument");
        *n = g->size();
    });
}

ocrs_status ocrs_engine_group_member(const ocrs_engine_group* g, size_t i, const ocrs_engine** engine, int* device) {
    return guarded([&] {
        if (!g || i >= g->size()) fail(OCRS_ERR_INVALID_ARGUMENT, "no such member");
        if (engine) *engine = g->members[i].engine.get();
        if (device) *device = g->members[i].device;
    });
}

ocrs_status ocrs_group_deal(size_t n_pages, size_t n_members, size_t min_block, size_t* member_of_page_out, size_t* pages_per_member) {
    return guarded([&] {
        if (n_members == 0 || (n_pages && !member_of_page_out)) fail(OCRS_ERR_INVALID_ARGUMENT, "bad argument");
        if (pages_per_member)
            for (size_t m = 0; m < n_members; m++) pages_per_member[m] = 0;
        const size_t b = block_size(n_pages, n_members, min_block ? min_block : 8);
        for (size_t i = 0; i < n_pages; i++) {
            const size_t m = (i / b) % n_members;
            member_of_page_out[i] = m;
            if (pages_per_member) pages_per_member[m]++;
        }
    });
}

ocrs_status ocrs_group_last_gather(const ocrs_engine_group* gc, int* transport, size_t* bytes, const char** why_host) {
    return guarded([&] {
        if (!gc) fail(OCRS_ERR_INVALID_ARGUMENT, "null argument");
        ocrs_engine_group* g = const_cast<ocrs_engine_group*>(gc);
        std::lock_guard<std::mutex> li(g->info_mu);
        if (transport) *transport = g->last_mode;
        if (bytes) *bytes = g->last_bytes;
        if (why_host) {
            g->why_host_out = g->why_host;
            *why_host = g->why_host_out.c_str();
        }
    });
}

static void group_prepare(ocrs_engine_group* g, const void* const* pixels, size_t n, bool on_device, ocrs_pixel_type type,
                          ocrs_dim_order order, int height, int width, int channels, ocrs_page** out) {
    if (!g || !out || (n > 0 && !pixels)) fail(OCRS_ERR_INVALID_ARGUMENT, "null argument");
    for (size_t i = 0; i < n; i++) check_image_args(pixels[i], height, width, channels);
    std::vector<std::vector<size_t>> of_member;
    if (on_device) {
        std::vector<size_t> dev(n);
        for (size_t i = 0; i < n; i++) {
            hipPointerAttribute_t attr;
            if (hipPointerGetAttributes(&attr, pixels[i]) != hipSuccess) {
                (void)hipGetLastError();
                fail(OCRS_ERR_INVALID_ARGUMENT, "image %zu: not a device pointer", i);
            }
            dev[i] = device_slot(g, attr.device);
            if (dev[i] == g->devices.size())
                fail(OCRS_ERR_INVALID_ARGUMENT, "image %zu lives on device %d, which has no member in this group", i, attr.device);
        }
        of_member = deal_resident(g, dev);
    } else {
        of_member = deal_free(g, n);
    }
    const size_t bytes = (size_t)height * width * channels * (type == OCRS_U8 ? 1 : 4);
    std::vector<std::unique_ptr<ocrs_page>> made(n);
    for_each_member(g, of_member, [&](size_t m) {
        const ocrs_engine* e = g->members[m].engine.get();
        if (g->replay_mode == 2) {
            for (size_t i : of_member[m]) {
                made[i] = new_page(height, width);
                made[i]->source = pixels[i];
            }
            std::this_thread::sleep_for(std::chrono::duration<double>(g->replay_s[0]));
            return;
        }
        Workspace ws;
        for (size_t i : of_member[m]) {
            const void* d_px = pixels[i];
            if (!on_device) {
                void* d = ws.alloc(bytes);
                OCRS_HIP(hipMemcpyAsync(d, pixels[i], bytes, hipMemcpyHostToDevice, ws.s()));
                d_px = d;
            }
            made[i].reset(make_page(d_px, type, order, height, width, channels, ws.s(), e->tm()));
            made[i]->source = pixels[i];
        }
        ws.sync();
        if (e->tm()) e->tm()->collect();
    });
    for (size_t i = 0; i < n; i++) out[i] = made[i].release();
}

ocrs_status ocrs_group_prepare_input_batch(const ocrs_engine_group* g, const void* const* pixels, size_t n, ocrs_pixel_type type,
                                           ocrs_dim_order order, int height, int width, int channels, ocrs_page** out) {
    return guarded([&] { group_prepare(const_cast<ocrs_engine_group*>(g), pixels, n, false, type, order, height, width, channels, out); });
}

ocrs_status ocrs_group_prepare_input_device_batch(const ocrs_engine_group* g, const void* const* d_pixels, size_t n,
                                                  ocrs_pixel_type type, ocrs_dim_order order, int height, int width, int channels,
                                                  ocrs_page** out) {
    return guarded([&] { group_prepare(const_cast<ocrs_engine_group*>(g), d_pixels, n, true, type, order, height, width, channels, out); });
}

static ocrs_status group_detect_words_batch(ocrs_engine_group* g, const ocrs_page* const* pages, size_t n_pages, float** rects,
                                            size_t* offsets, bool scored, float** score, uint32_t** pixels, int tile_overlap = -1) {
    return guarded([&] {
        if (!g || !rects || !offsets || (n_pages && !pages) || (scored && (!score || !pixels)))
            fail(OCRS_ERR_INVALID_ARGUMENT, "null argument");
        if (scored && g->replay_mode == 2) fail(OCRS_ERR_INVALID_ARGUMENT, "replay: detection scores are not recorded");
        if (tile_overlap >= 0 && g->replay_mode != 0) fail(OCRS_ERR_INVALID_ARGUMENT, "replay: tiled detection is not recorded");
        const auto of_member = deal_pages(g, pages, n_pages);
        const size_t G = g->size();
        std::vector<std::vector<uint8_t>> payloads(G);
        for_each_member(g, of_member, [&](size_t m) {
            std::vector<const ocrs_page*> mine;
            for (size_t i : of_member[m]) mine.push_back(pages[i]);
            std::vector<std::vector<RotatedRect>> rr;
            DetScores sc;
            if (g->replay_mode == 2) {
                {
                    std::lock_guard<std::mutex> lk(g->replay_mu);
                    for (const ocrs_page* pg : mine) {
                        auto it = g->replay_rects.find(pg->source);
                        if (it == g->replay_rects.end()) fail(OCRS_ERR_INVALID_ARGUMENT, "replay: no recorded detection for this page");
                        rr.push_back(it->second);
                    }
                }
                std::this_thread::sleep_for(std::chrono::duration<double>(g->replay_s[1]));
            } else {
                g->members[m].engine->detect(mine.data(), mine.size(), &rr, nullptr, scored ? &sc : nullptr, tile_overlap);
                if (g->replay_mode == 1) {
                    std::lock_guard<std::mutex> lk(g->replay_mu);
                    for (size_t j = 0; j < mine.size(); j++) g->replay_rects[mine[j]->source] = rr[j];
                }
            }
            auto& pl = payloads[m];
            std::vector<float> flat;
            for (size_t j = 0; j < rr.size(); j++) {
                const uint64_t cnt = rr[j].size();
                append_bytes(pl, &cnt, 1);
                flat.clear();
                append_rects(flat, rr[j]);
                append_bytes(pl, flat.data(), flat.size());
                if (scored) {
                    append_bytes(pl, sc.score[j].data(), cnt);
                    append_bytes(pl, sc.pixels[j].data(), cnt);
                }
            }
        });
        std::vector<size_t> moffs;
        const std::vector<uint8_t> all = gather_request(g, payloads, &moffs);
        std::vector<Cursor> cur = cursors(all, moffs);
        const std::vector<size_t> mo = member_of_page(of_member, n_pages);
        std::vector<float> flat, fscore;
        std::vector<uint32_t> fpixels;
        offsets[0] = 0;
        for (size_t i = 0; i < n_pages; i++) {
            Cursor& c = cur[mo[i]];
            const uint64_t cnt = c.count();
            if (cnt > (c.end - c.at) / ((scored ? 8 : 6) * sizeof(float))) c.need(SIZE_MAX);
            const float* src = reinterpret_cast<const float*>(c.take(cnt * 6 * sizeof(float)));
            flat.insert(flat.end(), src, src + cnt * 6);
            if (scored) {
                fscore.resize(fscore.size() + cnt);
                fpixels.resize(fpixels.size() + cnt);
                if (cnt) {
                    memcpy(fscore.data() + fscore.size() - cnt, c.take(cnt * sizeof(float)), cnt * sizeof(float));
// ... 226 lines not shown
```

ocrs_amd/csrc/kernels.hpp:

```cpp
#pragma once
#include <vector>
#include <hip/hip_runtime.h>

#include <cstdint>

namespace ocrs {
namespace jpeg { struct Coefficients; }
namespace k {

void prepare_image(const void* d_pixels, bool is_u8, bool chans_last, int h, int w, int chans, float* d_out,
                   hipStream_t s);
void resize_pages_to_model(const float* const* d_src_ptrs, int n, int sh, int sw, int vh, int vw, float* d_dst,
                           int dh, int dw, hipStream_t s);
bool resize_threshold(const float* d_prob, int n, int mh, int mw, int sh, int sw, float thr, uint8_t* d_mask,
                      float* d_map, int h, int w, hipStream_t s, int32_t* d_labels = nullptr, int32_t* d_zero_a = nullptr,
                      int32_t* d_zero_b = nullptr);
void threshold_only(const float* d_prob, float thr, uint8_t* d_mask, int64_t count, hipStream_t s);

struct CclBuffers {
    int32_t* labels;
    int32_t* row_counts;
    int32_t* row_offsets;
    int32_t* n_roots;
    int32_t* roots;
    int32_t* lengths;
    int32_t* offsets;
    int32_t* overflow;
    uint32_t* pts;
    uint32_t* tmp;
    uint8_t* keep;
    float* rects;
    uint8_t* valid;
    uint32_t* score_pixels;
    unsigned long long* score_sums;
};
void ccl_label(const uint8_t* d_mask, int n, int h, int w, const CclBuffers& b, int max_comp, hipStream_t s, bool prepared = false);
void contour_rects(const uint8_t* d_mask, int n, int h, int w, const CclBuffers& b, int max_comp, int64_t arena,
                   float expand, float min_area, float eps, hipStream_t s, bool prepared = false);

void component_scores(const uint8_t* d_mask, const float* d_map, int n, int h, int w, const CclBuffers& b, int max_comp,
                      hipStream_t s);

struct TileDesc {
    const float* page;
    uint8_t* mask;
    float* map;
    int32_t h, w;
    int32_t oy, ox;
    int32_t y0, y1, x0, x1;
};
void gather_tiles(const TileDesc* d_tiles, int n_tiles, float* d_dst, int mh, int mw, hipStream_t s);
void stitch_threshold(const TileDesc* d_tiles, int n_tiles, const float* d_prob, int mh, int mw, float thr, hipStream_t s);

struct GemmDesc {
    const float* A; int lda;
    const float* B; int ldb;
    const float* bias;
    float* C; int ldc;
    int M, N, K;
    int relu;
    int im2col; int H, W, Cin;
    int convt; int Cout;
    int batch; int64_t strideA, strideB, strideBias, strideC;
    int nfast = 0, nx = 0, ny = 0;
    const uint16_t* Bsplit = nullptr; int64_t strideBsplit = 0;
};
void gemm(const GemmDesc& d, hipStream_t s);
void conv_direct(const float* x, int n, int h, int w, int cin, const float* wt, const float* bias, int kh, int kw,
                 int cout, int relu, float* y, hipStream_t s);
void dwconv3x3(const float* x, int n, int h, int w, int c, const float* wt, const float* bias, int relu, float* y,
               hipStream_t s);
bool dwpw_fused_supported(int cin, int cout);
void dwpw_fused(const float* x, int n, int h, int w, int cin, const float* wdw, const float* bdw, int relu_dw, int cout,
                const float* wpw, const float* bpw, int relu_pw, float* y, hipStream_t s);
bool dwconv3x3_cat(const float* skip, int n, int h, int w, int cs, const float* up, int uh, int uw, int cu, const float* wt,
                   const float* bias, int relu, float* y, hipStream_t s);
struct DoubleConvArgs {
    const float* skip;
    const float* x1;
    const float *wt, *bt;
    const float *wd1, *bd1;
    const float *wp1, *bp1;
    const float *wd2, *bd2;
    const float *wp2, *bp2;
    const float *wf, *bf;
    float* y;
    float* ypool;
    int n, h, w, h1, w1;
    int relu_d1, relu_p1, relu_d2, relu_p2, sigmoid;
    int tiles_x, tiles_y;
    const float* tape = nullptr;
    int tape_len = 0;
    const float* rtape = nullptr;
    int rtape_len = 0;
// ... 205 lines not shown
```

ocrs_amd/csrc/kernels_image.hip:

```cpp
#include "bilinear.hpp"
#include "common.hpp"
#include "kernels.hpp"

namespace ocrs {
namespace k {

template <bool IS_U8, bool CHANS_LAST, int CHANS>
__global__ void __launch_bounds__(256) prepare_image_kernel(const void* __restrict__ src, float* __restrict__ out,
                                                            int64_t plane, float w0, float w1, float w2) {
    constexpr int NW = CHANS == 1 ? 1 : 3;
    const float wts[3] = {w0, w1, w2};
    const uint8_t* s8 = static_cast<const uint8_t*>(src);
    const float* sf = static_cast<const float*>(src);
    for (int64_t p = (int64_t)blockIdx.x * blockDim.x + threadIdx.x; p < plane;
         p += (int64_t)gridDim.x * blockDim.x) {
        float px = -0.5f;
#pragma unroll
        for (int c = 0; c < NW; c++) {
            int64_t idx = CHANS_LAST ? p * CHANS + c : (int64_t)c * plane + p;
            float v = IS_U8 ? (float)s8[idx] : sf[idx];
            px = px + v * wts[c];
        }
        out[p] = px;
    }
}

__global__ void __launch_bounds__(256) prepare_image_rgb8_x4_kernel(const uint32_t* __restrict__ src,
                                                                    float4* __restrict__ out, int64_t quads,
                                                                    float w0, float w1, float w2) {
    for (int64_t q = (int64_t)blockIdx.x * blockDim.x + threadIdx.x; q < quads;
         q += (int64_t)gridDim.x * blockDim.x) {
        uint32_t a = src[3 * q], b = src[3 * q + 1], c = src[3 * q + 2];
        float r0 = (float)(a & 0xff), g0 = (float)((a >> 8) & 0xff), b0 = (float)((a >> 16) & 0xff);
        float r1 = (float)(a >> 24), g1 = (float)(b & 0xff), b1 = (float)((b >> 8) & 0xff);
        float r2 = (float)((b >> 16) & 0xff), g2 = (float)(b >> 24), b2 = (float)(c & 0xff);
        float r3 = (float)((c >> 8) & 0xff), g3 = (float)((c >> 16) & 0xff), b3 = (float)(c >> 24);
        float4 o;
        o.x = ((-0.5f + r0 * w0) + g0 * w1) + b0 * w2;
        o.y = ((-0.5f + r1 * w0) + g1 * w1) + b1 * w2;
        o.z = ((-0.5f + r2 * w0) + g2 * w1) + b2 * w2;
        o.w = ((-0.5f + r3 * w0) + g3 * w1) + b3 * w2;
        out[q] = o;
    }
}

void prepare_image(const void* d_pixels, bool is_u8, bool chans_last, int h, int w, int chans, float* d_out,
                   hipStream_t s) {
    const float itu[3] = {0.299f, 0.587f, 0.114f};
    float wt[3];
    for (int c = 0; c < 3; c++) {
        if (chans == 1) wt[c] = is_u8 ? (1.0f / 255.0f) : 1.0f;
        else wt[c] = is_u8 ? (itu[c] / 255.0f) : itu[c];
    }
    const int64_t plane = (int64_t)h * w;
    if (is_u8 && chans_last && chans == 3 && plane % 4 == 0 && ((uintptr_t)d_pixels % 4) == 0 &&
        ((uintptr_t)d_out % 16) == 0) {
        int64_t quads = plane / 4;
        int grid = (int)((quads + 255) / 256 < 4096 ? (quads + 255) / 256 : 4096);
        hipLaunchKernelGGL(prepare_image_rgb8_x4_kernel, dim3(grid), dim3(256), 0, s, (const uint32_t*)d_pixels,
                           (float4*)d_out, quads, wt[0], wt[1], wt[2]);
        return;
    }
    int grid = (int)((plane + 255) / 256 < 8192 ? (plane + 255) / 256 : 8192);
    if (grid < 1) grid = 1;
#define LAUNCH(U8, CL, CH)                                                                                  \
    hipLaunchKernelGGL((prepare_image_kernel<U8, CL, CH>), dim3(grid), dim3(256), 0, s, d_pixels, d_out, plane, \
                       wt[0], wt[1], wt[2])
#define DISPATCH_CH(U8, CL)                  \
    switch (chans) {                         \
        case 1: LAUNCH(U8, CL, 1); break;    \
        case 3: LAUNCH(U8, CL, 3); break;    \
        default: LAUNCH(U8, CL, 4); break;   \
    }
    if (is_u8) {
        if (chans_last) { DISPATCH_CH(true, true) } else { DISPATCH_CH(true, false) }
    } else {
        if (chans_last) { DISPATCH_CH(false, true) } else { DISPATCH_CH(false, false) }
    }
#undef DISPATCH_CH
#undef LAUNCH
}

__global__ void __launch_bounds__(256)
resize_pages_kernel(const float* const* __restrict__ src_ptrs, int sh, int sw, int vh, int vw,
                    float* __restrict__ dst, int dh, int dw) {
    const int x = blockIdx.x * blockDim.x + threadIdx.x;
    const int y = blockIdx.y;
    const int n = blockIdx.z;
    if (x >= dw) return;
    const float* __restrict__ src = src_ptrs[n];
    int y0, y1, x0, x1;
    float wy, wx;
    resize_axis(y, vh, dh, y0, y1, wy);
    resize_axis(x, vw, dw, x0, x1, wx);
    const float fill = -0.5f;
    float tl = (y0 < sh && x0 < sw) ? src[(int64_t)y0 * sw + x0] : fill;
    float tr = (y0 < sh && x1 < sw) ? src[(int64_t)y0 * sw + x1] : fill;
    float bl = (y1 < sh && x0 < sw) ? src[(int64_t)y1 * sw + x0] : fill;
    float br = (y1 < sh && x1 < sw) ? src[(int64_t)y1 * sw + x1] : fill;
    dst[((int64_t)n * dh + y) * dw + x] = bilerp(tl, tr, bl, br, wx, wy);
}

void resize_pages_to_model(const float* const* d_src_ptrs, int n, int sh, int sw, int vh, int vw, float* d_dst,
                           int dh, int dw, hipStream_t s) {
    dim3 grid((dw + 255) / 256, dh, n);
    hipLaunchKernelGGL(resize_pages_kernel, grid, dim3(256), 0, s, d_src_ptrs, sh, sw, vh, vw, d_dst, dh, dw);
}

template <bool LABELS>
__global__ void __launch_bounds__(256)
resize_threshold_kernel(const float* __restrict__ prob, int mh, int mw, int sh, int sw, float thr,
                        uint8_t* __restrict__ mask, float* __restrict__ map, int h, int w, int32_t* __restrict__ labels,
                        int32_t* __restrict__ zero_a, int32_t* __restrict__ zero_b) {
    const int xq = blockIdx.x * blockDim.x + threadIdx.x;
    const int y = blockIdx.y;
    const int n = blockIdx.z;
    const int x_base = xq * 4;
    const bool inb = x_base < w;
    if (!LABELS && !inb) return;
    if (LABELS && xq == 0 && y == 0) { zero_a[n] = 0; zero_b[n] = 0; }
    const float* __restrict__ src = prob + (int64_t)n * mh * mw;
    int y0, y1;
    float wy;
    resize_axis(y, sh, h, y0, y1, wy);
    uint32_t bits = 0;
    float vals[4];
#pragma unroll
    for (int i = 0; i < 4; i++) {
        int x = x_base + i;
        float v = 0.0f;
        if (x < w) {
            int x0, x1;
            float wx;
            resize_axis(x, sw, w, x0, x1, wx);
            float tl = src[(int64_t)y0 * mw + x0], tr = src[(int64_t)y0 * mw + x1];
            float bl = src[(int64_t)y1 * mw + x0], br = src[(int64_t)y1 * mw + x1];
            v = bilerp(tl, tr, bl, br, wx, wy);
            if (v > thr) bits |= 1u << (8 * i);
        }
        vals[i] = v;
    }
    const int64_t o = ((int64_t)n * h + y) * w + x_base;
    if (LABELS) {
        const int lane = threadIdx.x & 63;
        const uint32_t cur = inb ? bits : 0x02020202u;
        const uint32_t prev = (uint32_t)__builtin_amdgcn_update_dpp(0, (int)cur, 0x138, 0xF, 0xF, true);
        const int v0 = cur & 0xFF, v1 = (cur >> 8) & 0xFF, v2 = (cur >> 16) & 0xFF, v3 = cur >> 24;
        const bool b0 = lane == 0 || v0 != (int)(prev >> 24), b1 = v1 != v0, b2 = v2 != v1, b3 = v3 != v2;
        const int top = b3 ? 3 : b2 ? 2 : b1 ? 1 : b0 ? 0 : -1;
        const unsigned long long any = __ballot(top >= 0);
        const unsigned long long below = any & ((1ull << lane) - 1ull);
        const int srcl = below ? 63 - __clzll(below) : 0;
        const int src_top = __shfl(top, srcl);
        if (!inb) return;
        const int seg = y * w + x_base - 4 * lane;
        const int carried = seg + 4 * srcl + src_top;
        int4 out;
        const int s0 = b0 ? seg + 4 * lane : carried;
        const int s1 = b1 ? seg + 4 * lane + 1 : s0;
        const int s2 = b2 ? seg + 4 * lane + 2 : s1;
        const int s3 = b3 ? seg + 4 * lane + 3 : s2;
        out.x = s0; out.y = s1; out.z = s2; out.w = s3;
        *reinterpret_cast<int4*>(labels + o) = out;
// ... 49 lines not shown
```

ocrs_amd/csrc/model.cpp:

```cpp
#include "model.hpp"

#include <cstdio>
#include <functional>
#include <map>
#include <mutex>

#include "kernels.hpp"

namespace ocrs {

namespace {
#pragma pack(push, 1)
struct FileHeader {
    char magic[8];
    uint32_t version, kind;
    int64_t input_shape[4];
    uint32_t n_ops, n_slots, out_slot, reserved;
    uint64_t blob_floats;
};
struct FileOp {
    uint32_t type;
    int32_t in0, in1, out, relu, kh, kw, cin, cout, hidden;
    uint32_t n_w, reserved;
    struct { uint64_t off, cnt; } w[8];
// ... 603 lines not shown
                break;
            }
            case OP_SIGMOID: timed(KC_OTHER, 0, 8.0 * a.count(), [&] { k::sigmoid(x, y, a.count(), st); }); break;
            case OP_TOSEQ:
                if (a.h != 1) fail(OCRS_ERR_RUN_FAILED, "model run failed: TOSEQ expects height 1, got %d", a.h);
                timed(KC_OTHER, 0, 8.0 * a.count(), [&] { k::to_seq(x, a.n, a.w, a.c, y, st); });
                break;
            case OP_GRU: {
                const int T = a.n, N = a.h, I = a.c, H = op.hidden;
                auto gx = get((size_t)2 * T * N * 3 * H);
                auto gh = get((size_t)2 * N * 3 * H);
                auto hs = get((size_t)2 * N * H);
                OCRS_HIP(hipMemsetAsync(hs.first, 0, (size_t)2 * N * H * sizeof(float), st));
                k::GemmDesc d{};
                d.A = x; d.lda = I; d.B = op.aux0; d.ldb = 3 * H; d.bias = op.aux1; d.C = gx.first; d.ldc = 3 * H;
                d.M = T * N; d.N = 3 * H; d.K = I; d.batch = 2;
                d.strideA = 0; d.strideB = (int64_t)I * 3 * H; d.strideBias = 3 * H; d.strideC = (int64_t)T * N * 3 * H;
                timed(KC_GEMM_GRU_INPUT, 2.0 * 2 * d.M * (double)d.N * d.K,
                      4.0 * ((double)a.count() + 2.0 * d.M * d.N + 2.0 * d.K * d.N), [&] { k::gemm(d, st); });
                k::GemmDesc r{};
                r.A = hs.first; r.lda = H; r.B = op.aux2; r.ldb = 3 * H; r.bias = op.aux3; r.C = gh.first; r.ldc = 3 * H;
                r.M = N; r.N = 3 * H; r.K = H; r.batch = 2;
                r.strideA = (int64_t)N * H; r.strideB = (int64_t)H * 3 * H; r.strideBias = 3 * H; r.strideC = (int64_t)N * 3 * H;
                for (int step = 0; step < T; step++) {
                    timed(KC_GEMM_GRU_HIDDEN, 2.0 * 2 * r.M * (double)r.N * r.K,
                          4.0 * 2 * ((double)r.M * r.K + (double)r.M * r.N + (double)r.K * r.N), [&] { k::gemm(r, st); });
                    timed(KC_GRU_GATES, 0, 4.0 * 2 * N * (double)H * 9,
                          [&] { k::gru_gates(gx.first, gh.first, hs.first, y, T, N, H, step, st); });
                }
                free_local.emplace(gx.second, gx.first);
                free_local.emplace(gh.second, gh.first);
                free_local.emplace(hs.second, hs.first);
                break;
            }
            case OP_LINEAR: {
                k::GemmDesc d{};
                d.A = x; d.lda = op.cin; d.B = op.w[0]; d.ldb = op.cout; d.bias = op.w[1];
                d.C = y; d.ldc = op.cout; d.M = (int)((int64_t)a.n * a.h * a.w); d.N = op.cout; d.K = op.cin;
                d.relu = op.relu;
                timed(KC_GEMM_LINEAR, 2.0 * d.M * (double)d.N * d.K, 4.0 * ((double)a.count() + o.count()) + wbytes(op, 0),
                      [&] { k::gemm(d, st); });
                break;
            }
            case OP_LOGSOFTMAX:
                timed(KC_LOGSOFTMAX_ARGMAX, 0, 4.0 * a.count() * (y ? 2.0 : 1.0), [&] {
                    if (!k::log_softmax_argmax(x, (int64_t)a.n * a.h * a.w, a.c, is_final_logsoftmax ? d_excluded : nullptr, y,
                                               is_final_logsoftmax ? d_labels : nullptr, st))
                        fail(OCRS_ERR_CAPACITY, "LogSoftmax over %d classes exceeds the kernel's LDS staging (max ~630)", a.c);
                });
                break;
            default: fail(OCRS_ERR_RUN_FAILED, "model run failed: bad op");
        }
        }
        if (print_timing) OCRS_HIP(hipEventRecord(ev[i + 1], st));
        for (int sl : {op.in0, op.in1}) {
            if (sl > 0 && last_use[sl] == (int)i && ptr[sl] && cap[sl]) {
                free_local.emplace(cap[sl], ptr[sl]);
                ptr[sl] = nullptr;
                cap[sl] = 0;
            }
        }
    }
    if (timers && cur_stage >= 0) timers->end(stage_token, st);
    OCRS_HIP(hipGetLastError());

    if (print_timing) {
        OCRS_HIP(hipStreamSynchronize(st));
        float total = 0.f;
        for (size_t i = 0; i < n_run; i++) {
            float ms = 0.f;
            (void)hipEventElapsedTime(&ms, ev[i], ev[i + 1]);
            total += ms;
            const TensorShape o = shp[ops[i].out];
            printf("%-10s [%d,%d,%d,%d] %.3fms\n", kOpNames[ops[i].type], o.n, o.h, o.w, o.c, ms);
        }
        printf("total %.3fms\n", total);
        for (auto& e : ev) (void)hipEventDestroy(e);
    }
    return ptr[ret_slot];
}

float* HipModel::run_prefix_ragged(Workspace& ws, hipStream_t exec, const std::vector<PackedGroup>& groups,
                                   const PackedPlan& plan, int h, int ts, StageTimers* timers, int* feat_c,
                                   const std::function<void()>& before_launch, const OpRange* range) const {
    const int G = (int)groups.size();
    if (G == 0 || ts <= 0) return nullptr;
    for (int i = 0; i < ts; i++) {
        const GraphOp& op = ops[i];
        if (op.in0 != (i == 0 ? 0 : ops[i - 1].out)) return nullptr;
        if (op.type == OP_CONV) {
            if (op.kh != 3 || op.kw != 3 || !op.relu) return nullptr;
            if (op.cin == 1) {
                if (i + 1 >= ts || ops[i + 1].type != OP_MAXPOOL || ops[i + 1].kh != 2 || ops[i + 1].kw != 2) return nullptr;
                if (op.cout > 64 || op.cout < 4 || (op.cout & (op.cout - 1)) != 0) return nullptr;
            } else if ((op.cin % 32) != 0 || op.cout < 64 || (op.cout % 4) != 0) {
                return nullptr;
            }
        } else if (op.type != OP_MAXPOOL && op.type != OP_AVGPOOL) {
            return nullptr;
        }
    }
    {
        int hh = h;
        for (int i = 0; i < ts; i++) {
            if (ops[i].type == OP_CONV && ops[i].cin != 1 && (hh % 4) != 0) return nullptr;
            if (ops[i].type == OP_MAXPOOL || ops[i].type == OP_AVGPOOL) hh /= ops[i].kh;
        }
    }
    for (int g = 0; g + 1 < G && !(range && range->first > 0); g++)
        if (groups[g].d_batch + (size_t)groups[g].n * h * groups[g].w != groups[g + 1].d_batch) return nullptr;

    hipStream_t st = exec;
    auto timed = [&](int cls, double flops, double bytes, auto&& launch) {
        int tok = timers ? timers->kbegin(cls, st, flops, bytes) : -1;
        launch();
        if (tok >= 0) timers->end(tok, st);
    };
    struct Geo { int H; std::vector<int32_t> W; };
    std::vector<Geo> geos;
    geos.push_back(Geo{h, {}});
    for (const PackedGroup& g : groups) geos[0].W.push_back(g.w);
    for (int i = 0; i < ts; i++) {
        Geo o = geos.back();
        if (ops[i].type == OP_MAXPOOL || ops[i].type == OP_AVGPOOL) {
            o.H /= ops[i].kh;
            for (auto& w : o.W) w /= ops[i].kw;
        }
        geos.push_back(std::move(o));
    }
    std::vector<int32_t> nvec;
    for (const PackedGroup& g : groups) nvec.push_back(g.n);
    std::vector<int32_t> meta32;
    std::vector<int64_t> meta64;
    struct GeoOff { size_t w, t128, t256, t32, t16, p, f32[2], f16[2], gap; int nt128, nt256, nt32, nt16, nf32[2], nf16[2], ngap; int64_t pixels; };
    std::vector<GeoOff> goff;
    const size_t n_at = 0;
    meta32.insert(meta32.end(), nvec.begin(), nvec.end());
    const size_t loff_at = meta32.size();
    {
        int32_t acc = 0;
        meta32.push_back(0);
        for (int g = 0; g < G; g++) { acc += nvec[g]; meta32.push_back(acc); }
    }
    for (const Geo& ge : geos) {
        GeoOff o{};
        o.w = meta32.size();
        meta32.insert(meta32.end(), ge.W.begin(), ge.W.end());
        o.t128 = meta32.size();
        int32_t a128 = 0, a256 = 0, a32 = 0, a16 = 0;
        int64_t px = 0;
        std::vector<int32_t> t256{0}, t32{0}, t16{0};
        std::vector<int32_t> f32[2] = {{0}, {0}}, f16[2] = {{0}, {0}};
        int32_t af32[2] = {0, 0}, af16[2] = {0, 0};
        std::vector<int32_t> tgap{0};
        int32_t agap = 0;
        std::vector<int64_t> pv{0};
        meta32.push_back(0);
        for (int g = 0; g < G; g++) {
            const int64_t rows = (int64_t)nvec[g] * ge.H * ge.W[g];
            a128 += (int32_t)((rows + 127) / 128);
            a256 += (int32_t)((rows + 255) / 256);
            a32 += nvec[g] * (ge.H / 4) * ((ge.W[g] + 31) / 32);
            a16 += nvec[g] * (ge.H / 8) * ((ge.W[g] + 15) / 16);
            agap += (int32_t)((ge.H / 8) * (((int64_t)nvec[g] * ((ge.W[g] + 2) & ~1) + 15) / 16));
            tgap.push_back(agap);
            for (int e = 0; e < 2; e++) {
                const int64_t cols = (int64_t)nvec[g] * (e ? (ge.W[g] + 1) & ~1 : ge.W[g]);
// ... 121 lines not shown
                      [&] { k::conv12_fused_ragged(cur, vin, vmid, op.w[0], op.w[1], op.cout, op2.w[0], op2.w[1], op2.cout, y2, vout, st, op2.wsplit); });
                y = y2;
                ybytes = (size_t)vout.pixels * op2.cout * sizeof(float);
                if (prev_buf) spare.emplace_back(prev_buf, prev_bytes);
                prev_buf = y;
                prev_bytes = ybytes;
                cur = y;
            }
            if (ok) {
                curC = op2.cout;
                i += 3;
                if (i >= last) { at = i; break; }
                continue;
            }
        }
        if (op.type == OP_CONV && op.cin == 1) {
            const k::RaggedView vout = view(i + 2);
            if ((run = launches(i, i + 1))) {
                ybytes = (size_t)vout.pixels * op.cout * sizeof(float);
                y = get((size_t)vout.pixels * op.cout);
                timed(KC_CONV_DIRECT, 2.0 * vin.pixels * 9 * op.cout, 4.0 * vin.pixels + 4.0 * vout.pixels * op.cout,
                      [&] { k::conv1_relu_pool_ragged(cur, vin, op.w[0], op.w[1], op.cout, y, vout, st); });
            }
            curC = op.cout;
            i += 1;
        } else if (op.type == OP_CONV) {
            const bool fuse = i + 1 < ts && ops[i + 1].type == OP_MAXPOOL && ops[i + 1].kh == 2 &&
                              (ops[i + 1].kw == 1 || ops[i + 1].kw == 2) && vin.H % 2 == 0;
            const int ph = fuse ? 2 : 1, pw = fuse ? ops[i + 1].kw : 1;
            const k::RaggedView vout = view(fuse ? i + 2 : i + 1);
            if ((run = launches(i, fuse ? i + 1 : i))) {
                ybytes = (size_t)vout.pixels * op.cout * sizeof(float);
                y = get((size_t)vout.pixels * op.cout);
                bool ok = false;
                timed(KC_GEMM_CONV3X3, 2.0 * vin.pixels * 9.0 * op.cin * op.cout,
                      4.0 * (vin.pixels * op.cin + vout.pixels * op.cout) + 4.0 * op.wcount[0],
                      [&] { ok = k::conv3x3_ragged(cur, vin, op.cin, op.w[0], op.w[1], op.cout, op.relu, ph, pw, y, vout, st, op.wsplit); });
                if (!ok) fail(OCRS_ERR_RUN_FAILED, "model run failed: ragged conv %d->%d at height %d not supported", op.cin, op.cout, vin.H);
            }
            curC = op.cout;
            if (fuse) i += 1;
        } else if (op.type == OP_AVGPOOL && i + 1 == ts && op.kw == 1 && op.kh == vin.H && (curC & 3) == 0) {
            launches(i, ts);
            break;
        } else if ((run = launches(i, i))) {
            const k::RaggedView vout = view(i + 1);
            ybytes = (size_t)vout.pixels * curC * sizeof(float);
            y = get((size_t)vout.pixels * curC);
            timed(KC_POOL, 0, 4.0 * curC * (vin.pixels + vout.pixels),
                  [&] { k::pool_ragged(cur, vin, curC, op.kh, op.kw, op.type == OP_AVGPOOL, y, vout, st); });
        }
        if (run) {
            if (prev_buf) spare.emplace_back(prev_buf, prev_bytes);
            prev_buf = y;
            prev_bytes = ybytes;
            cur = y;
        }
        if (i >= last) { at = i; break; }
    }
    float* X = nullptr;
    if (at < ts) {
        X = ws.alloc_n<float>(prev_bytes / sizeof(float));
        OCRS_HIP(hipMemcpyAsync(X, prev_buf, prev_bytes, hipMemcpyDeviceToDevice, st));
    } else {
        const k::RaggedView vf = view(ts);
        if (vf.H != 1) fail(OCRS_ERR_RUN_FAILED, "model run failed: TOSEQ expects height 1, got %d", vf.H);
        X = ws.alloc_n<float>((size_t)plan.R * curC);
        const bool pool_here = ts >= 1 && ops[ts - 1].type == OP_AVGPOOL && ops[ts - 1].kw == 1 && (curC & 3) == 0 &&
                               ops[ts - 1].kh == view(ts - 1).H;
        if (pool_here) {
            const k::RaggedView vp = view(ts - 1);
            timed(KC_POOL, 0, 4.0 * curC * (vp.pixels + vf.pixels),
                  [&] { k::avgpool_to_seq_ragged(cur, vp, vf, curC, groups[0].d_pos, plan.d_off, X, st); });
        } else {
            launches(ts, ts);
            timed(KC_OTHER, 0, 8.0 * vf.pixels * curC,
                  [&] { k::to_seq_packed_ragged(cur, vf, curC, groups[0].d_pos, plan.d_off, X, st); });
        }
    }
    if (tok >= 0) timers->end(tok, st);
    if (exec != ws.s()) {
        hipEvent_t done = ws.make_event();
        OCRS_HIP(hipEventRecord(done, exec));
        OCRS_HIP(hipStreamWaitEvent(ws.s(), done, 0));
    }
    *feat_c = curC;
    return X;
}

const int32_t* HipModel::make_packed_plan(Workspace& ws, const std::vector<int32_t>& T, PackedPlan* plan,
                                          std::vector<size_t>* order) {
    order->clear();
    for (size_t i = 0; i < T.size(); i++)
        if (T[i] > 0) order->push_back(i);
    std::stable_sort(order->begin(), order->end(), [&](size_t a, size_t b) { return T[a] > T[b]; });
    const int M = (int)order->size();
    if (M == 0) return nullptr;
    plan->M = M;
    plan->Tmax = T[(*order)[0]];
    plan->active.assign(plan->Tmax, 0);
    std::vector<int32_t> hTm(M), hoff(plan->Tmax + 1, 0), hpos(T.size(), 0);
    for (int m = 0; m < M; m++) {
        hTm[m] = T[(*order)[m]];
        hpos[(*order)[m]] = m;
        for (int t = 0; t < hTm[m]; t++) plan->active[t]++;
    }
    for (int t = 0; t < plan->Tmax; t++) hoff[t + 1] = hoff[t] + plan->active[t];
    plan->R = hoff[plan->Tmax];
    std::vector<int32_t> meta(hTm);
    meta.insert(meta.end(), hoff.begin(), hoff.end());
    meta.insert(meta.end(), hpos.begin(), hpos.end());
    int32_t* d_meta = ws.alloc_n<int32_t>(meta.size());
    ws.upload(d_meta, meta.data(), meta.size() * sizeof(int32_t));
    plan->d_Tm = d_meta;
    plan->d_off = d_meta + M;
    plan->h_Tm = std::move(hTm);
    plan->h_off = std::move(hoff);
    return d_meta + M + plan->Tmax + 1;
}

int HipModel::packed_split() const {
    int ts = -1;
    for (size_t i = 0; i < ops.size(); i++)
        if (ops[i].type == OP_TOSEQ) { ts = (int)i; break; }
    if (ts < 0 || (size_t)ts + 3 > ops.size()) return -1;
    int prev_out = ops[ts].out;
    for (size_t i = ts + 1; i < ops.size(); i++) {
        const GraphOp& op = ops[i];
        const bool last = i + 1 == ops.size(), second_last = i + 2 == ops.size();
        if (op.in0 != prev_out) return -1;
        if (last) { if (op.type != OP_LOGSOFTMAX || (uint32_t)op.out != out_slot) return -1; }
        else if (second_last) { if (op.type != OP_LINEAR) return -1; }
        else if (op.type != OP_GRU) return -1;
        prev_out = op.out;
    }
    for (int i = 0; i < ts; i++)
        if (ops[i].type == OP_GRU || ops[i].type == OP_LINEAR || ops[i].type == OP_LOGSOFTMAX || ops[i].type == OP_TOSEQ)
            return -1;
    return ts;
}

int HipModel::run_recognition_packed(Workspace& ws, const std::vector<PackedGroup>& groups, const PackedPlan& plan, int h,
                                     StageTimers* timers, const uint8_t* d_excluded, int32_t* d_labels,
                                     float** d_logp, float* d_maxlp, OpRange* range) const {
    const int ts = packed_split();
    if (ts < 0) fail(OCRS_ERR_RUN_FAILED, "model run failed: graph is not <conv stack> TOSEQ GRU* LINEAR LOGSOFTMAX");
    const int first = range ? range->first : 0, last = range ? range->last : (int)ops.size() - 1;
    hipStream_t st = ws.s();
    auto timed = [&](int cls, double flops, double bytes, auto&& launch) {
        int tok = timers ? timers->kbegin(cls, st, flops, bytes) : -1;
        launch();
        if (tok >= 0) timers->end(tok, st);
    };
    const int64_t R = plan.R;
    const int M = plan.M;

    float* X = nullptr;
    int C0 = 0;
    if (first <= ts) {
        std::unique_lock<std::mutex> heavy(ctx().heavy_phase, std::defer_lock);
        const hipStream_t conv = ws.stream.conv_stream();
        try {
            X = run_prefix_ragged(ws, conv, groups, plan, h, ts, timers, &C0, [&] { heavy.lock(); }, range);
        } catch (...) {
            hipEvent_t e = nullptr;
            if (hipEventCreateWithFlags(&e, hipEventDisableTiming) == hipSuccess) {
                ws.events.push_back(e);
                if (hipEventRecord(e, conv) != hipSuccess || hipStreamWaitEvent(ws.s(), e, 0) != hipSuccess)
                    (void)hipStreamSynchronize(conv);
            } else {
                (void)hipStreamSynchronize(conv);
            }
            throw;
        }
    }
    if (range && first <= ts) {
        if (!X) fail(OCRS_ERR_INVALID_ARGUMENT, "op range: this model's conv stack has no ragged form");
        if (last < ts) {
            range->out = X;
            range->out_c = C0;
            return 0;
        }
    }
    if (!X && first <= ts)
    for (const PackedGroup& g : groups) {
        TensorShape fs;
        float* feat = run_device(ws, g.d_batch, g.n, h, g.w, &fs, timers, nullptr, nullptr, true, false, ts);
        if (fs.h != 1) fail(OCRS_ERR_RUN_FAILED, "model run failed: TOSEQ expects height 1, got %d", fs.h);
        if (!X) {
            C0 = fs.c;
            X = ws.alloc_n<float>((size_t)R * C0);
        }
        int tok = timers ? timers->begin(ST_REC_CONV, st, 0) : -1;
        timed(KC_OTHER, 0, 8.0 * fs.count(), [&] { k::to_seq_packed(feat, g.n, fs.w, fs.c, g.d_pos, plan.d_off, X, st); });
        if (tok >= 0) timers->end(tok, st);
    }
    if (!X && first <= ts) return 0;

    const float* cur = first <= ts ? X : range->seq_in;
    int curC = first <= ts ? C0 : range->in_c;
    int classes = 0;
    int gru_layer = 0;
    float* gx_buf = nullptr;
    size_t gx_cap = 0;
    void* hx_buf = nullptr;
    size_t hx_cap = 0;
    for (int i = std::max(ts + 1, first); i <= last; i++) {
        const GraphOp& op = ops[i];
        if (op.type == OP_GRU) {
            const int H = op.hidden, I = op.cin;
            if (I != curC) fail(OCRS_ERR_RUN_FAILED, "model run failed: GRU input size %d != %d", I, curC);
            int tok = timers ? timers->begin(ST_REC_GRU, st, 0) : -1;
            const size_t gx_floats = (size_t)2 * R * 3 * H;
            if (gx_floats > gx_cap) { gx_buf = ws.alloc_n<float>(gx_floats); gx_cap = gx_floats; }
            float* gx = gx_buf;
            float* y = ws.alloc_n<float>((size_t)R * 2 * H);
            const bool fused = (H == 256 || H == 128 || H == 64);
            const bool persistent = fused && gru_mode() == GRU_PERSISTENT && k::gru_persistent_supported(plan.h_Tm.data(), M, plan.Tmax, R, H);
            const int np = option(OPT_NUMERICS) == 1 ? 3 : option(OPT_NUMERICS) == 2 ? 2 : 0;
            const bool split = persistent && np != 0 && k::gru_split_supported(plan.h_Tm.data(), M, plan.Tmax, R, H, np);
            const size_t hx_bytes = split ? k::gru_split_exchange_bytes(plan.h_Tm.data(), M, H, np) : persistent ? k::gru_persistent_exchange_bytes(plan.h_Tm.data(), M, H) : 0;
            if (hx_bytes > hx_cap) { hx_buf = ws.alloc(hx_bytes); hx_cap = hx_bytes; }
            uint16_t* hx = split ? static_cast<uint16_t*>(hx_buf) : nullptr;
            float* hxf = persistent && !split ? static_cast<float*>(hx_buf) : nullptr;
            if (split) OCRS_HIP(k::gru_split_prepare(hx, plan.h_Tm.data(), M, H, np, st));
            else if (persistent) OCRS_HIP(k::gru_persistent_prepare(hxf, plan.h_Tm.data(), M, H, st));
            k::GemmDesc d{};
            d.A = cur; d.lda = I; d.B = op.aux0; d.ldb = 3 * H; d.bias = op.aux1; d.C = gx; d.ldc = 3 * H;
            d.M = (int)R; d.N = 3 * H; d.K = I; d.batch = 2;
            d.strideA = 0; d.strideB = (int64_t)I * 3 * H; d.strideBias = 3 * H; d.strideC = R * 3 * H;
            d.Bsplit = op.wsplit; d.strideBsplit = (int64_t)(3 * H / 128) * (I / 16) * 3 * 128 * 16;
            const double gx_flops = 2.0 * 2 * R * (double)d.N * d.K, gx_bytes = 4.0 * ((double)R * I + 2.0 * R * d.N + 2.0 * d.K * d.N);
            timed(KC_GEMM_GRU_INPUT, gx_flops, gx_bytes, [&] { k::gemm(d, st); });
            if (range && range->gx_only && i == last) {
                range->out = gx;
                range->out_c = 3 * H;
                return 0;
            }
            bool ran_persistent = false;
            if (persistent) {
                uint32_t* d_sync = ws.alloc_n<uint32_t>(k::gru_persistent_sync_words(M));
                double fl = 0.0;
                for (int step = 0; step < plan.Tmax; step++) fl += 2.0 * 2 * plan.active[step] * 3.0 * H * H;
                {
                    DeviceContext& dc = ctx();
                    std::lock_guard<std::mutex> g(dc.rec_phase);
                    hipStream_t rs = ws.stream.recurrent_stream();
                    hipEvent_t ready = ws.make_event(), done = ws.make_event();
                    OCRS_HIP(hipEventRecord(ready, st));
                    OCRS_HIP(hipStreamWaitEvent(rs, ready, 0));
                    int ktok = timers ? timers->kbegin(KC_GEMM_GRU_HIDDEN, rs, fl, 4.0 * ((double)R * (2.0 * 3 * H + 2.0 * 2 * H) + 2.0 * 3 * H * H)) : -1;
                    ran_persistent = split ? k::gru_persistent_split(gx, op.aux2, op.aux3, y, hx, plan.d_Tm, plan.d_off, plan.h_Tm.data(), R, M, plan.Tmax, H, np, d_sync, rs)
                                           : k::gru_persistent(gx, op.aux2, op.aux3, y, hxf, plan.d_Tm, plan.d_off, plan.h_Tm.data(), R, M, plan.Tmax, H, d_sync, rs);
                    if (ktok >= 0) timers->end(ktok, rs);
                    if (ran_persistent && plan.h_status && gru_layer < 8)
                        ws.download(plan.h_status + gru_layer, d_sync + k::gru_persistent_sync_words(M) - 1, sizeof(uint32_t), rs);
                    OCRS_HIP(hipEventRecord(done, rs));
                    OCRS_HIP(hipStreamWaitEvent(st, done, 0));
                }
            }
            if (ran_persistent) {
            } else if (fused) {
                const int Mcap = (M + 3) & ~3;
                float* hT0 = ws.alloc_n<float>((size_t)2 * H * Mcap);
                float* hT1 = ws.alloc_n<float>((size_t)2 * H * Mcap);
                OCRS_HIP(hipMemsetAsync(hT0, 0, (size_t)2 * H * Mcap * sizeof(float), st));
                for (int step = 0; step < plan.Tmax; step++) {
                    const int act = plan.active[step];
                    if (act <= 0) break;
                    const float* hin = (step & 1) ? hT1 : hT0;
                    float* hout = (step & 1) ? hT0 : hT1;
                    timed(KC_GEMM_GRU_HIDDEN, 2.0 * 2 * act * 3.0 * H * H,
                          4.0 * 2 * ((double)act * H * 2 + (double)act * 3 * H + 3.0 * H * H + (double)act * H), [&] {
                              if (!k::gru_step_fused(gx, op.aux2, op.aux3, hin, hout, y, plan.d_Tm, plan.d_off, R, Mcap, act, H, step, st))
                                  fail(OCRS_ERR_RUN_FAILED, "model run failed: no fused GRU step kernel for hidden size %d", H);
                          });
                }
            } else {
                float* gh = ws.alloc_n<float>((size_t)2 * M * 3 * H);
                float* hs = ws.alloc_n<float>((size_t)2 * M * H);
                OCRS_HIP(hipMemsetAsync(hs, 0, (size_t)2 * M * H * sizeof(float), st));
                k::GemmDesc r{};
                r.A = hs; r.lda = H; r.B = op.aux2; r.ldb = 3 * H; r.bias = op.aux3; r.C = gh; r.ldc = 3 * H;
                r.N = 3 * H; r.K = H; r.batch = 2;
                r.strideA = (int64_t)M * H; r.strideB = (int64_t)H * 3 * H; r.strideBias = 3 * H; r.strideC = (int64_t)M * 3 * H;
                for (int step = 0; step < plan.Tmax; step++) {
                    const int act = plan.active[step];
                    if (act <= 0) break;
                    r.M = act;
                    timed(KC_GEMM_GRU_HIDDEN, 2.0 * 2 * act * (double)r.N * r.K,
                          4.0 * 2 * ((double)act * r.K + (double)act * r.N + (double)r.K * r.N), [&] { k::gemm(r, st); });
                    timed(KC_GRU_GATES, 0, 4.0 * 2 * act * (double)H * 9, [&] {
                        k::gru_gates_packed(gx, gh, hs, y, plan.d_Tm, plan.d_off, R, M, act, H, step, st);
                    });
                }
            }
            if (tok >= 0) timers->end(tok, st);
            gru_layer++;
            cur = y;
            curC = 2 * H;
        } else if (op.type == OP_LINEAR) {
            if (op.cin != curC) fail(OCRS_ERR_RUN_FAILED, "model run failed: Linear input size %d != %d", op.cin, curC);
            int tok = timers ? timers->begin(ST_REC_HEAD, st, 0) : -1;
            float* y = ws.alloc_n<float>((size_t)R * op.cout);
            k::GemmDesc d{};
            d.A = cur; d.lda = op.cin; d.B = op.w[0]; d.ldb = op.cout; d.bias = op.w[1];
            d.C = y; d.ldc = op.cout; d.M = (int)R; d.N = op.cout; d.K = op.cin; d.relu = op.relu;
            timed(KC_GEMM_LINEAR, 2.0 * R * (double)d.N * d.K, 4.0 * ((double)R * (op.cin + op.cout)) + 4.0 * op.wcount[0],
                  [&] { k::gemm(d, st); });
            if (tok >= 0) timers->end(tok, st);
            cur = y;
            curC = op.cout;
        } else {
            int tok = timers ? timers->begin(ST_REC_HEAD, st, 0) : -1;
            float* lp = nullptr;
            if (d_logp || range) {
                lp = ws.alloc_n<float>((size_t)R * curC);
                if (d_logp) *d_logp = lp;
            }
            timed(KC_LOGSOFTMAX_ARGMAX, 0, 4.0 * R * curC * (lp ? 2.0 : 1.0),
                  [&] {
                      if (!k::log_softmax_argmax(cur, R, curC, d_excluded, lp, d_labels, st, d_maxlp))
                          fail(OCRS_ERR_CAPACITY, "LogSoftmax over %d classes exceeds the kernel's LDS staging (max ~630)", curC);
                  });
            if (tok >= 0) timers->end(tok, st);
            classes = curC;
            if (range) cur = lp;
        }
    }
    if (range) {
        range->out = cur;
        range->out_c = curC;
    }
    OCRS_HIP(hipGetLastError());
    return classes;
}

}
```

ocrs_amd/csrc/model.hpp:

```cpp
#pragma once
#include <functional>
#include <memory>
#include <string>
#include <vector>

#include "common.hpp"

namespace ocrs {

enum OpType : uint32_t {
    OP_CONV = 0, OP_DWCONV3, OP_MAXPOOL, OP_AVGPOOL, OP_CONVT2, OP_PADCAT, OP_SIGMOID, OP_TOSEQ, OP_GRU, OP_LINEAR,
    OP_LOGSOFTMAX, OP_COUNT
};

struct GraphOp {
    uint32_t type;
    int32_t in0, in1, out;
    int32_t relu, kh, kw, cin, cout, hidden;
    const float* w[8] = {nullptr};
    size_t wcount[8] = {0};
    const float* aux0 = nullptr;
    const float* aux1 = nullptr;
    const float* aux2 = nullptr;
    const float* aux3 = nullptr;
// ... 6 lines not shown
    int dc_block = -1;
};

struct DcBlock {
    int first = -1, last = -1;
    int convt = -1, cat = -1, dw1 = -1, pw1 = -1, dw2 = -1, pw2 = -1, pool = -1, fin = -1, sig = -1;
    int cs = 0, cx = 0, cmid = 0, cout = 0;
    const float* tape = nullptr;
    int tape_len = 0;
    const float* rtape = nullptr;
    int rtape_len = 0;
};

struct TensorShape {
    int n = 0, h = 0, w = 0, c = 0;
    bool seq = false;
    int64_t count() const { return (int64_t)n * h * w * c; }
};

struct ModelBase {
    virtual ~ModelBase() = default;
    int device = -1;
    int64_t input_shape[4] = {-1, -1, -1, -1};
    virtual bool is_callback() const = 0;
};

struct CallbackModel : ModelBase {
    ocrs_model_run_fn fn = nullptr;
    void* user = nullptr;
    bool is_callback() const override { return true; }
    void run(const float* input, const int64_t in_shape[4], std::vector<float>& out, int64_t out_shape[4],
             int* out_ndim) const;
};

struct HipModel : ModelBase {
    uint32_t kind = 0;
    std::vector<GraphOp> ops;
    std::vector<DcBlock> dc_blocks;
    uint32_t n_slots = 0, out_slot = 0;
    DevBuf weights;
    std::vector<DevBuf> tapes;
    bool is_callback() const override { return false; }

    static std::unique_ptr<HipModel> load(const void* data, size_t len, int device = -1);

    TensorShape infer(int n, int h, int w, std::vector<TensorShape>* slots = nullptr) const;
    double flops(int n, int h, int w) const;

    float* run_device(Workspace& ws, const float* d_in, int n, int h, int w, TensorShape* out_shape,
                      StageTimers* timers, const uint8_t* d_excluded = nullptr, int32_t* d_labels = nullptr,
                      bool want_logp = true, bool print_timing = false, int stop_before = -1,
                      hipStream_t exec = nullptr ) const;

    int packed_split() const;
    struct PackedGroup {
        const float* d_batch;
        int n, w;
        const int32_t* d_pos;
    };
    struct PackedPlan {
        int M = 0, Tmax = 0;
        int64_t R = 0;
        const int32_t* d_Tm = nullptr;
        const int32_t* d_off = nullptr;
        std::vector<int> active;
        std::vector<int32_t> h_Tm;
        std::vector<int32_t> h_off;
        uint32_t* h_status = nullptr;
    };
    struct OpRange {
        int first = 0, last = 0;
        bool gx_only = false;
        const float* seq_in = nullptr;
        int in_c = 0;
        const float* out = nullptr;
        int out_c = 0;
    };
    static const int32_t* make_packed_plan(Workspace& ws, const std::vector<int32_t>& T, PackedPlan* plan, std::vector<size_t>* order);
    int run_recognition_packed(Workspace& ws, const std::vector<PackedGroup>& groups, const PackedPlan& plan, int h,
                               StageTimers* timers, const uint8_t* d_excluded, int32_t* d_labels,
                               float** d_logp = nullptr, float* d_maxlp = nullptr, OpRange* range = nullptr) const;
    float* run_prefix_ragged(Workspace& ws, hipStream_t exec, const std::vector<PackedGroup>& groups,
                             const PackedPlan& plan, int h, int ts, StageTimers* timers, int* feat_c,
                             const std::function<void()>& before_launch = nullptr, const OpRange* range = nullptr) const;
};

}

struct ocrs_model {
    std::unique_ptr<ocrs::ModelBase> impl;
};
```

Measured before the change: 272.1.

## Cap per-device stream count with lane plan, batch page preparation, host-wait joins

Adds a LanePlan that bounds leased streams to a fixed budget of shared light lanes, assigned least-loaded, instead of creating a private stream per lease. Lease completion events now come from a reused pool. Page preparation for a batch is launched as one multi-page kernel instead of a kernel per page. Cross-stream joins after the conv stack and the recurrent phase can become host waits, so the heavy lock is released earlier. The aim is less stream and launch overhead and less contention, at the risk of serialising work on shared lanes and adding host blocking.

```diff
diff --git a/include/ocrs_amd.h b/include/ocrs_amd.h
--- a/include/ocrs_amd.h
+++ b/include/ocrs_amd.h
@@ -48,6 +48,8 @@
 
 OCRS_API ocrs_status ocrs_coalescer_selftest(int n_threads, int requests_per_thread, int max_active, int max_pages,
                                              long window_us, int fail_every, uint64_t out[5]);
+
+OCRS_API ocrs_status ocrs_stream_plan_selftest(int budget, const int32_t* ops, size_t n_ops, int32_t* out);
 
 OCRS_API ocrs_status ocrs_set_option(const char* name, long value);
 OCRS_API ocrs_status ocrs_option_name(int index, const char** name);
diff --git a/ocrs_amd/_lib.py b/ocrs_amd/_lib.py
--- a/ocrs_amd/_lib.py
+++ b/ocrs_amd/_lib.py
@@ -62,7 +62,7 @@
     "ocrs_get_device", "ocrs_model_load_file_on_device", "ocrs_model_load_bytes_on_device", "ocrs_model_device", "ocrs_engine_device",
     "ocrs_engine_group_new", "ocrs_engine_group_free", "ocrs_engine_group_size", "ocrs_engine_group_member", "ocrs_group_deal",
     "ocrs_group_prepare_input_batch", "ocrs_group_prepare_input_device_batch", "ocrs_group_detect_words_batch",
-    "ocrs_group_recognize_text_batch", "ocrs_group_gather", "ocrs_group_final_gather", "ocrs_group_worker_threads", "ocrs_group_last_gather", "ocrs_device_malloc_on", "ocrs_engine_coalesce_stats", "ocrs_coalescer_selftest", "ocrs_engine_kernel_mfma_flops", "ocrs_engine_prepare_input_jpeg", "ocrs_jpeg_decode_rgb", "ocrs_jpeg_info", "ocrs_jpeg_coefficients",
+    "ocrs_group_recognize_text_batch", "ocrs_group_gather", "ocrs_group_final_gather", "ocrs_group_worker_threads", "ocrs_group_last_gather", "ocrs_device_malloc_on", "ocrs_engine_coalesce_stats", "ocrs_coalescer_selftest", "ocrs_stream_plan_selftest", "ocrs_engine_kernel_mfma_flops", "ocrs_engine_prepare_input_jpeg", "ocrs_jpeg_decode_rgb", "ocrs_jpeg_info", "ocrs_jpeg_coefficients",
     "ocrs_group_member_stats", "ocrs_numa_parse_cpulist", "ocrs_numa_bind_selftest", "ocrs_engine_recognize_logits", "ocrs_engine_set_option", "ocrs_engine_get_option", "ocrs_option_name", "ocrs_device_pool_stats", "ocrs_device_pool_configure", "ocrs_device_pool_trim",
     "ocrs_device_set_isolation", "ocrs_device_isolation", "ocrs_group_set_replay", "ocrs_abi_version",
     "ocrs_engine_recognize_text_scored", "ocrs_engine_recognize_text_batch_scored", "ocrs_ctc_beam_search_scored",
diff --git a/ocrs_amd/csrc/abi.cpp b/ocrs_amd/csrc/abi.cpp
--- a/ocrs_amd/csrc/abi.cpp
+++ b/ocrs_amd/csrc/abi.cpp
@@ -62,6 +62,25 @@
     return guarded([&] {
         if (!out || n_threads < 1 || requests_per_thread < 1 || max_pages < 1) fail(OCRS_ERR_INVALID_ARGUMENT, "bad argument");
         coalescer_selftest(n_threads, requests_per_thread, max_active, max_pages, window_us, fail_every, out);
+    });
+}
+
+ocrs_status ocrs_stream_plan_selftest(int budget, const int32_t* ops, size_t n_ops, int32_t* out) {
+    return guarded([&] {
+        if (!out || (n_ops > 0 && !ops) || !LanePlan::valid_budget(budget)) fail(OCRS_ERR_INVALID_ARGUMENT, "bad argument");
+        LanePlan plan(budget);
+        for (size_t i = 0; i < n_ops; i++) {
+            const int32_t op = ops[2 * i], arg = ops[2 * i + 1];
+            switch (op) {
+                case 0: out[i] = plan.acquire(arg); break;
+                case 1: plan.release(arg); out[i] = plan.outstanding(); break;
+                case 2: out[i] = plan.set_budget(arg) ? 1 : 0; break;
+                case 3: out[i] = plan.load(arg); break;
+                case 4: out[i] = plan.budget(); break;
+                case 5: out[i] = plan.light_lanes(); break;
+                default: fail(OCRS_ERR_INVALID_ARGUMENT, "unknown op %d", (int)op);
+            }
+        }
     });
 }
 
@@ -152,6 +171,8 @@
 static void check_option_set(int r, const char* name, long value) {
     if (r == 1) fail(OCRS_ERR_INVALID_ARGUMENT, "unknown option '%s'", name ? name : "(null)");
     if (r == 2) fail(OCRS_ERR_INVALID_ARGUMENT, "option '%s': value %ld is out of range", name, value);
+    if (r == 3) fail(OCRS_ERR_INVALID_ARGUMENT, "option '%s' cannot change while a request is in flight on a device", name);
+    if (r == 4) fail(OCRS_ERR_INVALID_ARGUMENT, "option '%s' belongs to the devices, not to an engine: set it with ocrs_set_option", name);
 }
 
 ocrs_status ocrs_set_option(const char* name, long value) {
@@ -399,12 +420,13 @@
         for (size_t i = 0; i < n; i++) check_image_args(pixels[i], height, width, channels);
         Workspace ws;
         const size_t bytes = (size_t)height * width * channels * (type == OCRS_U8 ? 1 : 4);
-        std::vector<std::unique_ptr<ocrs_page>> made;
+        std::vector<const void*> d_px(n);
         for (size_t i = 0; i < n; i++) {
-            void* d_px = ws.alloc(bytes);
-            OCRS_HIP(hipMemcpyAsync(d_px, pixels[i], bytes, hipMemcpyHostToDevice, ws.s()));
-            made.emplace_back(make_page(d_px, type, order, height, width, channels, ws.s(), e->tm()));
-        }
+            void* d = ws.alloc(bytes);
+            OCRS_HIP(hipMemcpyAsync(d, pixels[i], bytes, hipMemcpyHostToDevice, ws.s()));
+            d_px[i] = d;
+        }
+        std::vector<std::unique_ptr<ocrs_page>> made = make_pages(d_px.data(), n, type, order, height, width, channels, ws.s(), e->tm());
         ws.sync();
         if (e->tm()) e->tm()->collect();
         for (size_t i = 0; i < n; i++) out[i] = made[i].release();
diff --git a/ocrs_amd/csrc/abi_util.cpp b/ocrs_amd/csrc/abi_util.cpp
--- a/ocrs_amd/csrc/abi_util.cpp
+++ b/ocrs_amd/csrc/abi_util.cpp
@@ -63,6 +63,22 @@
     return page.release();
 }
 
+std::vector<std::unique_ptr<ocrs_page>> make_pages(const void* const* d_pixels, size_t n, ocrs_pixel_type type, ocrs_dim_order order,
+                                                   int height, int width, int channels, hipStream_t st, StageTimers* T) {
+    std::vector<std::unique_ptr<ocrs_page>> made;
+    std::vector<float*> outs;
+    for (size_t i = 0; i < n; i++) {
+        made.push_back(new_page(height, width));
+        outs.push_back(made.back()->grey.as<float>());
+    }
+    if (n) {
+        StageScope sc(T, ST_PREPARE, st, (n + k::PrepareTable::kPages - 1) / k::PrepareTable::kPages);
+        k::prepare_image_batch(d_pixels, outs.data(), (int)n, type == OCRS_U8, order == OCRS_HWC, height, width, channels, st);
+    }
+    OCRS_HIP(hipGetLastError());
+    return made;
+}
+
 void check_image_args(const void* pixels, int height, int width, int channels) {
     if (!pixels) fail(OCRS_ERR_INVALID_ARGUMENT, "pixels is null");
     if (!(channels == 1 || channels == 3 || channels == 4)) fail(OCRS_ERR_IMAGE_SOURCE, "channel count is not 1, 3 or 4");
diff --git a/ocrs_amd/csrc/abi_util.hpp b/ocrs_amd/csrc/abi_util.hpp
--- a/ocrs_amd/csrc/abi_util.hpp
+++ b/ocrs_amd/csrc/abi_util.hpp
@@ -102,6 +102,8 @@
 std::vector<std::vector<geom::RotatedRect>> unpack_lines(const float* rects, const size_t* offsets, size_t first, size_t last);
 ocrs_page* make_page(const void* d_pixels, ocrs_pixel_type type, ocrs_dim_order order, int height, int width, int channels,
                      hipStream_t st, StageTimers* T);
+std::vector<std::unique_ptr<ocrs_page>> make_pages(const void* const* d_pixels, size_t n, ocrs_pixel_type type, ocrs_dim_order order,
+                                                   int height, int width, int channels, hipStream_t st, StageTimers* T);
 void check_image_args(const void* pixels, int height, int width, int channels);
 std::unique_ptr<ocrs_engine> make_engine(const ocrs_engine_params& params);
 void flatten_chars(const ocrs_engine* e, const std::vector<RecResult>& res, std::vector<ocrs_text_char>* flat, std::vector<size_t>* offs);
diff --git a/ocrs_amd/csrc/common.cpp b/ocrs_amd/csrc/common.cpp
--- a/ocrs_amd/csrc/common.cpp
+++ b/ocrs_amd/csrc/common.cpp
@@ -38,6 +38,14 @@
         g_ctx[device].store(c, std::memory_order_release);
     }
     return *c;
+}
+
+static bool any_device_has_calls_in_flight() {
+    for (auto& slot : g_ctx) {
+        DeviceContext* c = slot.load(std::memory_order_acquire);
+        if (c && c->calls_in_flight()) return true;
+    }
+    return false;
 }
 
 int default_device() { return g_default_device.load(); }
@@ -313,27 +321,47 @@
     return st;
 }
 
+void DeviceContext::create_lanes_locked(int n_light) {
+    if (heavy_ && recurrent_ && (int)light_.size() >= n_light) return;
+    DeviceScope bind(device);
+    int least = 0, greatest = 0;
+    OCRS_HIP(hipDeviceGetStreamPriorityRange(&least, &greatest));
+    if (!heavy_) OCRS_HIP(hipStreamCreateWithPriority(&heavy_, hipStreamNonBlocking, greatest));
+    if (!recurrent_) OCRS_HIP(hipStreamCreateWithPriority(&recurrent_, hipStreamNonBlocking, greatest));
+    while ((int)light_.size() < n_light) {
+        hipStream_t s = nullptr;
+        OCRS_HIP(hipStreamCreateWithPriority(&s, hipStreamNonBlocking, greatest));
+        light_.push_back(s);
+    }
+}
+
+int DeviceContext::planned_light_lanes() {
+    (void)plan.set_budget((int)process_option(OPT_STREAM_BUDGET));
+    return plan.light_lanes();
+}
+
 hipStream_t DeviceContext::heavy_stream() {
     std::lock_guard<std::mutex> g(lazy_mu_);
-    if (!heavy_) {
-        DeviceScope bind(device);
-        int least = 0, greatest = 0;
-        OCRS_HIP(hipDeviceGetStreamPriorityRange(&least, &greatest));
-        OCRS_HIP(hipStreamCreateWithPriority(&heavy_, hipStreamNonBlocking, greatest));
-    }
+    create_lanes_locked(planned_light_lanes());
     return heavy_;
 }
 
 hipStream_t DeviceContext::recurrent_stream(int mode) {
     if (mode == MODE_SERIAL) return heavy_stream();
     std::lock_guard<std::mutex> g(lazy_mu_);
-    if (!recurrent_) {
-        DeviceScope bind(device);
-        int least = 0, greatest = 0;
-        OCRS_HIP(hipDeviceGetStreamPriorityRange(&least, &greatest));
-        OCRS_HIP(hipStreamCreateWithPriority(&recurrent_, hipStreamNonBlocking, greatest));
-    }
+    create_lanes_locked(planned_light_lanes());
     return recurrent_;
+}
+
+hipStream_t DeviceContext::light_lane(int lane) {
+    std::lock_guard<std::mutex> g(lazy_mu_);
+    create_lanes_locked(std::max(lane + 1, plan.light_lanes()));
+    return light_[lane];
+}
+
+bool DeviceContext::calls_in_flight() {
+    std::lock_guard<std::mutex> lk(iso_mu_);
+    return leases_ > 0;
 }
 
 static thread_local int t_lease_depth[kMaxDevices] = {0};
@@ -416,6 +444,7 @@
     {"conv_flat", "OCRS_CONV_FLAT", 1},
     {"beam_gpu", "OCRS_BEAM_GPU", 1},
     {"det_tile_batch", "OCRS_DET_TILE_BATCH", 16},
+    {"stream_budget", "OCRS_STREAM_BUDGET", LanePlan::kDefaultBudget},
     {"numerics", nullptr, 0},
     {"coalesce", nullptr, 2},
     {"coalesce_pages", nullptr, 16},
@@ -426,11 +455,12 @@
 struct OptRange { long lo, hi; long also[4]; };
 const OptRange kOptRanges[OPT_COUNT] = {
     {0, 1, {}}, {0, 1, {}}, {0, 1, {}}, {0, 2, {}}, {0, 1, {8, 14, 32}}, {0, 1, {8, 14, 20, 32}}, {0, 1, {}}, {0, 1, {}}, {0, 1, {}}, {0, 1, {}},
-    {1, 1024, {}},
+    {1, 1024, {}}, {LanePlan::kMinBudget, LanePlan::kMaxBudget, {}},
     {0, 2, {}}, {0, 64, {}}, {1, 4096, {}}, {0, 10000000, {}}, {0, 4096, {}}, {0, INT64_MAX, {}},
 };
 bool in_range(int i, long v) {
     const OptRange& r = kOptRanges[i];
+    if (i == OPT_STREAM_BUDGET) return LanePlan::valid_budget(v);
     if (v >= r.lo && v <= r.hi) return true;
     for (long a : r.also) if (a && v == a) return true;
     return false;
@@ -458,6 +488,11 @@
 TuningScope::~TuningScope() { t_tuning = prev_; }
 const Tuning* current_tuning() { return t_tuning; }
 
+long process_option(Option o) {
+    std::call_once(g_opts_once, init_options);
+    return g_opts[o].load(std::memory_order_relaxed);
+}
+
 long option_long(Option o) {
     if (t_tuning) return __atomic_load_n(&t_tuning->v[o], __ATOMIC_RELAXED);
     std::call_once(g_opts_once, init_options);
@@ -482,6 +517,7 @@
         return 1;
     }
     if (!in_range(i, value)) return 2;
+    if (i == OPT_STREAM_BUDGET && value != g_opts[i].load() && any_device_has_calls_in_flight()) return 3;
     g_opts[i].store(value);
     return 0;
 }
@@ -489,6 +525,7 @@
 int set_option(Tuning& t, const char* name, long value) {
     const int i = find_option(name, OPT_COUNT);
     if (i < 0) return 1;
+    if (i == OPT_STREAM_BUDGET) return 4;
     if (!in_range(i, value)) return 2;
     __atomic_store_n(&t.v[i], value, __ATOMIC_RELAXED);
     return 0;
@@ -501,22 +538,42 @@
     return true;
 }
 
-StreamLease::StreamLease(bool high_priority) : ctx_(&ctx()), high_(high_priority) {
+static hipEvent_t take_lease_event(DeviceContext* c) {
+    {
+        std::lock_guard<std::mutex> g(c->stream_mu);
+        if (!c->lease_events.empty()) {
+            hipEvent_t e = c->lease_events.back();
+            c->lease_events.pop_back();
+            return e;
+        }
+    }
+    hipEvent_t e = nullptr;
+    OCRS_HIP(hipEventCreateWithFlags(&e, hipEventBlockingSync | hipEventDisableTiming));
+    return e;
+}
+
+StreamLease::StreamLease(bool high_priority, int avoid_lane) : ctx_(&ctx()), high_(high_priority) {
     high_ = true;
     mode_ = ctx_->lease_begin();
     try {
+        done_ = take_lease_event(ctx_);
         if (mode_ == DeviceContext::MODE_SERIAL) {
             s_ = ctx_->heavy_stream();
             shared_ = true;
-            OCRS_HIP(hipEventCreateWithFlags(&done_, hipEventBlockingSync | hipEventDisableTiming));
+            return;
+        }
+        (void)ctx_->planned_light_lanes();
+        lane_ = ctx_->plan.acquire(avoid_lane);
+        counted_ = true;
+        if (lane_ >= 0) {
+            s_ = ctx_->light_lane(lane_);
             return;
         }
         {
             std::lock_guard<std::mutex> g(ctx_->stream_mu);
             auto& v = ctx_->streams;
             if (!v.empty()) {
-                s_ = v.back().first;
-                done_ = v.back().second;
+                s_ = v.back();
                 v.pop_back();
                 return;
             }
@@ -524,20 +581,24 @@
         int least = 0, greatest = 0;
         OCRS_HIP(hipDeviceGetStreamPriorityRange(&least, &greatest));
         OCRS_HIP(hipStreamCreateWithPriority(&s_, hipStreamNonBlocking, greatest));
-        OCRS_HIP(hipEventCreateWithFlags(&done_, hipEventBlockingSync | hipEventDisableTiming));
     } catch (...) {
+        if (counted_) ctx_->plan.release(lane_);
+        if (done_) {
+            std::lock_guard<std::mutex> g(ctx_->stream_mu);
+            ctx_->lease_events.push_back(done_);
+        }
         ctx_->lease_end();
         throw;
     }
 }
 
 StreamLease::~StreamLease() {
-    if (shared_) {
-        (void)hipEventDestroy(done_);
-    } else {
+    {
         std::lock_guard<std::mutex> g(ctx_->stream_mu);
-        ctx_->streams.emplace_back(s_, done_);
-    }
+        ctx_->lease_events.push_back(done_);
+        if (!shared_ && lane_ < 0) ctx_->streams.push_back(s_);
+    }
+    if (counted_) ctx_->plan.release(lane_);
     ctx_->lease_end();
 }
 
diff --git a/ocrs_amd/csrc/common.hpp b/ocrs_amd/csrc/common.hpp
--- a/ocrs_amd/csrc/common.hpp
+++ b/ocrs_amd/csrc/common.hpp
@@ -17,6 +17,7 @@
 #include <vector>
 
 #include "../../include/ocrs_amd.h"
+#include "stream_plan.hpp"
 
 namespace ocrs {
 
@@ -100,7 +101,12 @@
     int cu_count();
     std::vector<struct DevBuf> heavy_arena;
     std::mutex stream_mu;
-    std::vector<std::pair<hipStream_t, hipEvent_t>> streams;
+    LanePlan plan;
+    std::vector<hipStream_t> streams;
+    std::vector<hipEvent_t> lease_events;
+    hipStream_t light_lane(int lane);
+    int planned_light_lanes();
+    bool calls_in_flight();
 
     explicit DeviceContext(int d) : device(d), pool(d) {}
 
@@ -109,6 +115,8 @@
     template <class F> void switch_isolation(F&& change);
     std::mutex lazy_mu_;
     hipStream_t heavy_ = nullptr, recurrent_ = nullptr;
+    std::vector<hipStream_t> light_;
+    void create_lanes_locked(int n_light);
     int cus_ = 0;
     std::mutex iso_mu_;
     std::condition_variable iso_cv_;
@@ -140,7 +148,7 @@
 inline hipStream_t heavy_stream() { return ctx().heavy_stream(); }
 
 enum Option { OPT_GRU_MODE = 0, OPT_GRU_GATES, OPT_GRU_LOCAL, OPT_DET_FUSE, OPT_DET_STREAM, OPT_DET_ROWS, OPT_CCL_QUAD,
-              OPT_CONV12_FUSE, OPT_CONV_FLAT, OPT_BEAM_GPU, OPT_DET_TILE_BATCH, OPT_PUBLIC_COUNT,
+              OPT_CONV12_FUSE, OPT_CONV_FLAT, OPT_BEAM_GPU, OPT_DET_TILE_BATCH, OPT_STREAM_BUDGET, OPT_PUBLIC_COUNT,
               OPT_NUMERICS = OPT_PUBLIC_COUNT,
               OPT_COALESCE, OPT_COALESCE_PAGES, OPT_COALESCE_WINDOW_US,
               OPT_LAYOUT_THREADS, OPT_REC_MAX_PIXELS,
@@ -163,6 +171,7 @@
 const Tuning* current_tuning();
 enum { GRU_PERSISTENT = 0, GRU_STEP = 1 };
 int option(Option o);
+long process_option(Option o);
 
 inline void allow_dynamic_lds(const void* kernel, std::atomic<uint64_t>& done) {
     int dev = 0;
@@ -205,20 +214,25 @@
     template <class T> T* as() const { return static_cast<T*>(p); }
 };
 
+inline hipError_t wait_event(hipEvent_t ev) noexcept {
+    for (int i = 0;; i++) {
+        const hipError_t e = hipEventQuery(ev);
+        if (e != hipErrorNotReady) return e;
+        if (i < 64) std::this_thread::yield();
+        else std::this_thread::sleep_for(std::chrono::microseconds(i < 256 ? 20 : 100));
+    }
+}
+
 class StreamLease {
   public:
-    explicit StreamLease(bool high_priority = false);
+    explicit StreamLease(bool high_priority = false, int avoid_lane = LanePlan::kPrivate);
     ~StreamLease();
     hipStream_t get() const { return s_; }
+    int lane() const { return lane_; }
+    bool may_park_waits() const { return lane_ < 0 || ctx_->plan.outstanding() <= 1; }
     hipError_t wait_done() const noexcept {
-        hipError_t e = hipEventRecord(done_, s_);
-        if (e != hipSuccess) return e;
-        for (int i = 0;; i++) {
-            e = hipEventQuery(done_);
-            if (e != hipErrorNotReady) return e;
-            if (i < 64) std::this_thread::yield();
-            else std::this_thread::sleep_for(std::chrono::microseconds(i < 256 ? 20 : 100));
-        }
+        const hipError_t e = hipEventRecord(done_, s_);
+        return e != hipSuccess ? e : wait_event(done_);
     }
     void sync() const { OCRS_HIP(wait_done()); }
     hipError_t sync_noexcept() const noexcept { return wait_done(); }
@@ -231,8 +245,10 @@
     DeviceContext* ctx_;
     DeviceContext::Mode mode_ = DeviceContext::MODE_FREE;
     bool shared_ = false;
-    hipStream_t s_;
-    hipEvent_t done_;
+    bool counted_ = false;
+    int lane_ = LanePlan::kPrivate;
+    hipStream_t s_ = nullptr;
+    hipEvent_t done_ = nullptr;
     bool high_;
 };
 
@@ -301,12 +317,13 @@
     std::vector<hipEvent_t> events;
     hipEvent_t make_event() {
         hipEvent_t e;
-        OCRS_HIP(hipEventCreateWithFlags(&e, hipEventDisableTiming));
+        OCRS_HIP(hipEventCreateWithFlags(&e, hipEventBlockingSync | hipEventDisableTiming));
         events.push_back(e);
         return e;
     }
     Workspace() = default;
-    explicit Workspace(bool high_priority) : stream(high_priority) {}
+    explicit Workspace(bool high_priority, int avoid_lane = LanePlan::kPrivate) : stream(high_priority, avoid_lane) {}
+    void host_wait(hipEvent_t ev) { OCRS_HIP(wait_event(ev)); }
     std::vector<void*> upload_staging;
     void upload(void* d_dst, const void* h_src, size_t bytes) {
         if (!bytes) return;
diff --git a/ocrs_amd/csrc/engine.cpp b/ocrs_amd/csrc/engine.cpp
--- a/ocrs_amd/csrc/engine.cpp
+++ b/ocrs_amd/csrc/engine.cpp
@@ -1,6 +1,7 @@
 #include "engine.hpp"
 
 #include <algorithm>
+#include <exception>
 #include <limits>
 #include <map>
 #include <thread>
@@ -1177,18 +1178,41 @@
     size_t n_long_lines = 0, n_short_lines = 0;
     for (size_t c = 0; c < chunks.size(); c++) (c >= first_long ? n_long_lines : n_short_lines) += chunks[c].members.size();
     const bool split = n_long_lines > 0 && n_short_lines >= 64;
-    Workspace ws_long(true);
     Sub sub_long, sub_short;
     if (split) {
-        {
+        Workspace ws_long(true, ws.stream.lane());
+        if (ws_long.s() != ws.s()) {
             hipEvent_t crops = ws.make_event();
             OCRS_HIP(hipEventRecord(crops, ws.s()));
             OCRS_HIP(hipStreamWaitEvent(ws_long.s(), crops, 0));
         }
-        launch_packed(rq, first_long, chunks.size(), ws_long, sub_long);
-        launch_packed(rq, 0, first_long, ws, sub_short);
-        ws_long.sync();
-        ws.sync();
+        if (ws.stream.may_park_waits()) {
+            launch_packed(rq, first_long, chunks.size(), ws_long, sub_long);
+            launch_packed(rq, 0, first_long, ws, sub_short);
+            ws_long.sync();
+            ws.sync();
+        } else {
+            std::exception_ptr long_error;
+            const Tuning* tuning = current_tuning();
+            const int device = ctx().device;
+            std::thread long_thread([&] {
+                try {
+                    DeviceScope bind(device);
+                    TuningScope tune(tuning);
+                    launch_packed(rq, first_long, chunks.size(), ws_long, sub_long);
+                    ws_long.sync();
+                    if (StageTimers* T = e.tm()) T->collect();
+                } catch (...) {
+                    long_error = std::current_exception();
+                }
+                StageTimers::release_thread_events();
+            });
+            struct Join { std::thread& t; ~Join() { if (t.joinable()) t.join(); } } join{long_thread};
+            launch_packed(rq, 0, first_long, ws, sub_short);
+            ws.sync();
+            long_thread.join();
+            if (long_error) std::rethrow_exception(long_error);
+        }
         unpack_packed(rq, sub_long);
         unpack_packed(rq, sub_short);
     } else {
diff --git a/ocrs_amd/csrc/group.cpp b/ocrs_amd/csrc/group.cpp
--- a/ocrs_amd/csrc/group.cpp
+++ b/ocrs_amd/csrc/group.cpp
@@ -543,14 +543,19 @@
             return;
         }
         Workspace ws;
+        std::vector<const void*> d_px;
         for (size_t i : of_member[m]) {
-            const void* d_px = pixels[i];
+            d_px.push_back(pixels[i]);
             if (!on_device) {
                 void* d = ws.alloc(bytes);
                 OCRS_HIP(hipMemcpyAsync(d, pixels[i], bytes, hipMemcpyHostToDevice, ws.s()));
-                d_px = d;
-            }
-            made[i].reset(make_page(d_px, type, order, height, width, channels, ws.s(), e->tm()));
+                d_px.back() = d;
+            }
+        }
+        auto share = make_pages(d_px.data(), d_px.size(), type, order, height, width, channels, ws.s(), e->tm());
+        for (size_t j = 0; j < share.size(); j++) {
+            const size_t i = of_member[m][j];
+            made[i] = std::move(share[j]);
             made[i]->source = pixels[i];
         }
         ws.sync();
diff --git a/ocrs_amd/csrc/kernels.hpp b/ocrs_amd/csrc/kernels.hpp
--- a/ocrs_amd/csrc/kernels.hpp
+++ b/ocrs_amd/csrc/kernels.hpp
@@ -10,6 +10,13 @@
 
 void prepare_image(const void* d_pixels, bool is_u8, bool chans_last, int h, int w, int chans, float* d_out,
                    hipStream_t s);
+struct PrepareTable {
+    enum { kPages = 32 };
+    const void* src[kPages];
+    float* dst[kPages];
+};
+void prepare_image_batch(const void* const* d_pixels, float* const* d_out, int n, bool is_u8, bool chans_last, int h, int w,
+                         int chans, hipStream_t s);
 void resize_pages_to_model(const float* const* d_src_ptrs, int n, int sh, int sw, int vh, int vw, float* d_dst,
                            int dh, int dw, hipStream_t s);
 bool resize_threshold(const float* d_prob, int n, int mh, int mw, int sh, int sw, float thr, uint8_t* d_mask,
diff --git a/ocrs_amd/csrc/kernels_image.hip b/ocrs_amd/csrc/kernels_image.hip
--- a/ocrs_amd/csrc/kernels_image.hip
+++ b/ocrs_amd/csrc/kernels_image.hip
@@ -6,8 +6,8 @@
 namespace k {
 
 template <bool IS_U8, bool CHANS_LAST, int CHANS>
-__global__ void __launch_bounds__(256) prepare_image_kernel(const void* __restrict__ src, float* __restrict__ out,
-                                                            int64_t plane, float w0, float w1, float w2) {
+__device__ __forceinline__ void prepare_pixels(const void* __restrict__ src, float* __restrict__ out, int64_t plane, float w0,
+                                               float w1, float w2) {
     constexpr int NW = CHANS == 1 ? 1 : 3;
     const float wts[3] = {w0, w1, w2};
     const uint8_t* s8 = static_cast<const uint8_t*>(src);
@@ -25,9 +25,8 @@
     }
 }
 
-__global__ void __launch_bounds__(256) prepare_image_rgb8_x4_kernel(const uint32_t* __restrict__ src,
-                                                                    float4* __restrict__ out, int64_t quads,
-                                                                    float w0, float w1, float w2) {
+__device__ __forceinline__ void prepare_quads_rgb8(const uint32_t* __restrict__ src, float4* __restrict__ out, int64_t quads,
+                                                   float w0, float w1, float w2) {
     for (int64_t q = (int64_t)blockIdx.x * blockDim.x + threadIdx.x; q < quads;
          q += (int64_t)gridDim.x * blockDim.x) {
         uint32_t a = src[3 * q], b = src[3 * q + 1], c = src[3 * q + 2];
@@ -44,17 +43,46 @@
     }
 }
 
-void prepare_image(const void* d_pixels, bool is_u8, bool chans_last, int h, int w, int chans, float* d_out,
-                   hipStream_t s) {
+template <bool IS_U8, bool CHANS_LAST, int CHANS>
+__global__ void __launch_bounds__(256) prepare_image_kernel(const void* __restrict__ src, float* __restrict__ out,
+                                                            int64_t plane, float w0, float w1, float w2) {
+    prepare_pixels<IS_U8, CHANS_LAST, CHANS>(src, out, plane, w0, w1, w2);
+}
+
+__global__ void __launch_bounds__(256) prepare_image_rgb8_x4_kernel(const uint32_t* __restrict__ src,
+                                                                    float4* __restrict__ out, int64_t quads,
+                                                                    float w0, float w1, float w2) {
+    prepare_quads_rgb8(src, out, quads, w0, w1, w2);
+}
+
+template <bool IS_U8, bool CHANS_LAST, int CHANS>
+__global__ void __launch_bounds__(256) prepare_image_batch_kernel(PrepareTable t, int64_t plane, float w0, float w1, float w2) {
+    prepare_pixels<IS_U8, CHANS_LAST, CHANS>(t.src[blockIdx.y], t.dst[blockIdx.y], plane, w0, w1, w2);
+}
+
+__global__ void __launch_bounds__(256) prepare_image_rgb8_x4_batch_kernel(PrepareTable t, int64_t quads, float w0, float w1, float w2) {
+    prepare_quads_rgb8(static_cast<const uint32_t*>(t.src[blockIdx.y]), reinterpret_cast<float4*>(t.dst[blockIdx.y]), quads, w0, w1, w2);
+}
+
+namespace {
+void prepare_weights(bool is_u8, int chans, float wt[3]) {
     const float itu[3] = {0.299f, 0.587f, 0.114f};
-    float wt[3];
     for (int c = 0; c < 3; c++) {
         if (chans == 1) wt[c] = is_u8 ? (1.0f / 255.0f) : 1.0f;
         else wt[c] = is_u8 ? (itu[c] / 255.0f) : itu[c];
     }
+}
+bool prepare_x4_ok(const void* d_pixels, bool is_u8, bool chans_last, int chans, int64_t plane, const float* d_out) {
+    return is_u8 && chans_last && chans == 3 && plane % 4 == 0 && ((uintptr_t)d_pixels % 4) == 0 && ((uintptr_t)d_out % 16) == 0;
+}
+}
+
+void prepare_image(const void* d_pixels, bool is_u8, bool chans_last, int h, int w, int chans, float* d_out,
+                   hipStream_t s) {
+    float wt[3];
+    prepare_weights(is_u8, chans, wt);
     const int64_t plane = (int64_t)h * w;
-    if (is_u8 && chans_last && chans == 3 && plane % 4 == 0 && ((uintptr_t)d_pixels % 4) == 0 &&
-        ((uintptr_t)d_out % 16) == 0) {
+    if (prepare_x4_ok(d_pixels, is_u8, chans_last, chans, plane, d_out)) {
         int64_t quads = plane / 4;
         int grid = (int)((quads + 255) / 256 < 4096 ? (quads + 255) / 256 : 4096);
         hipLaunchKernelGGL(prepare_image_rgb8_x4_kernel, dim3(grid), dim3(256), 0, s, (const uint32_t*)d_pixels,
@@ -79,6 +107,43 @@
     }
 #undef DISPATCH_CH
 #undef LAUNCH
+}
+
+void prepare_image_batch(const void* const* d_pixels, float* const* d_out, int n, bool is_u8, bool chans_last, int h, int w,
+                         int chans, hipStream_t s) {
+    float wt[3];
+    prepare_weights(is_u8, chans, wt);
+    const int64_t plane = (int64_t)h * w;
+    bool x4 = true;
+    for (int i = 0; i < n; i++) x4 = x4 && prepare_x4_ok(d_pixels[i], is_u8, chans_last, chans, plane, d_out[i]);
+    for (int i0 = 0; i0 < n; i0 += PrepareTable::kPages) {
+        const int m = n - i0 < (int)PrepareTable::kPages ? n - i0 : (int)PrepareTable::kPages;
+        PrepareTable t{};
+        for (int i = 0; i < m; i++) { t.src[i] = d_pixels[i0 + i]; t.dst[i] = d_out[i0 + i]; }
+        if (x4) {
+            const int64_t quads = plane / 4;
+            const int gx = (int)((quads + 255) / 256 < 4096 ? (quads + 255) / 256 : 4096);
+            hipLaunchKernelGGL(prepare_image_rgb8_x4_batch_kernel, dim3(gx, m), dim3(256), 0, s, t, quads, wt[0], wt[1], wt[2]);
+            continue;
+        }
+        int gx = (int)((plane + 255) / 256 < 8192 ? (plane + 255) / 256 : 8192);
+        if (gx < 1) gx = 1;
+#define LAUNCH(U8, CL, CH) \
+    hipLaunchKernelGGL((prepare_image_batch_kernel<U8, CL, CH>), dim3(gx, m), dim3(256), 0, s, t, plane, wt[0], wt[1], wt[2])
+#define DISPATCH_CH(U8, CL)                  \
+    switch (chans) {                         \
+        case 1: LAUNCH(U8, CL, 1); break;    \
+        case 3: LAUNCH(U8, CL, 3); break;    \
+        default: LAUNCH(U8, CL, 4); break;   \
+    }
+        if (is_u8) {
+            if (chans_last) { DISPATCH_CH(true, true) } else { DISPATCH_CH(true, false) }
+        } else {
+            if (chans_last) { DISPATCH_CH(false, true) } else { DISPATCH_CH(false, false) }
+        }
+#undef DISPATCH_CH
+#undef LAUNCH
+    }
 }
 
 __global__ void __launch_bounds__(256)
diff --git a/ocrs_amd/csrc/model.cpp b/ocrs_amd/csrc/model.cpp
--- a/ocrs_amd/csrc/model.cpp
+++ b/ocrs_amd/csrc/model.cpp
@@ -709,7 +709,8 @@
 
 float* HipModel::run_prefix_ragged(Workspace& ws, hipStream_t exec, const std::vector<PackedGroup>& groups,
                                    const PackedPlan& plan, int h, int ts, StageTimers* timers, int* feat_c,
-                                   const std::function<void()>& before_launch, const OpRange* range) const {
+                                   const std::function<void()>& before_launch, const OpRange* range,
+                                   hipEvent_t* stack_done) const {
     const int G = (int)groups.size();
     if (G == 0 || ts <= 0) return nullptr;
     for (int i = 0; i < ts; i++) {
@@ -997,7 +998,8 @@
     if (exec != ws.s()) {
         hipEvent_t done = ws.make_event();
         OCRS_HIP(hipEventRecord(done, exec));
-        OCRS_HIP(hipStreamWaitEvent(ws.s(), done, 0));
+        if (stack_done && !ws.stream.may_park_waits()) *stack_done = done;
+        else OCRS_HIP(hipStreamWaitEvent(ws.s(), done, 0));
     }
     *feat_c = curC;
     return X;
@@ -1075,19 +1077,20 @@
     if (first <= ts) {
         std::unique_lock<std::mutex> heavy(ctx().heavy_phase, std::defer_lock);
         const hipStream_t conv = ws.stream.conv_stream();
+        hipEvent_t stack_done = nullptr;
         try {
-            X = run_prefix_ragged(ws, conv, groups, plan, h, ts, timers, &C0, [&] { heavy.lock(); }, range);
+            X = run_prefix_ragged(ws, conv, groups, plan, h, ts, timers, &C0, [&] { heavy.lock(); }, range, &stack_done);
         } catch (...) {
             hipEvent_t e = nullptr;
-            if (hipEventCreateWithFlags(&e, hipEventDisableTiming) == hipSuccess) {
-                ws.events.push_back(e);
-                if (hipEventRecord(e, conv) != hipSuccess || hipStreamWaitEvent(ws.s(), e, 0) != hipSuccess)
-                    (void)hipStreamSynchronize(conv);
-            } else {
-                (void)hipStreamSynchronize(conv);
-            }
+            const bool recorded = hipEventCreateWithFlags(&e, hipEventBlockingSync | hipEventDisableTiming) == hipSuccess &&
+                                  hipEventRecord(e, conv) == hipSuccess;
+            if (e) ws.events.push_back(e);
+            if (heavy.owns_lock()) heavy.unlock();
+            if (!recorded || wait_event(e) != hipSuccess) (void)hipStreamSynchronize(conv);
             throw;
         }
+        if (heavy.owns_lock()) heavy.unlock();
+        if (stack_done) ws.host_wait(stack_done);
     }
     if (range && first <= ts) {
         if (!X) fail(OCRS_ERR_INVALID_ARGUMENT, "op range: this model's conv stack has no ragged form");
@@ -1157,6 +1160,7 @@
                 uint32_t* d_sync = ws.alloc_n<uint32_t>(k::gru_persistent_sync_words(M));
                 double fl = 0.0;
                 for (int step = 0; step < plan.Tmax; step++) fl += 2.0 * 2 * plan.active[step] * 3.0 * H * H;
+                hipEvent_t rec_done = nullptr;
                 {
                     DeviceContext& dc = ctx();
                     std::lock_guard<std::mutex> g(dc.rec_phase);
@@ -1171,8 +1175,10 @@
                     if (ran_persistent && plan.h_status && gru_layer < 8)
                         ws.download(plan.h_status + gru_layer, d_sync + k::gru_persistent_sync_words(M) - 1, sizeof(uint32_t), rs);
                     OCRS_HIP(hipEventRecord(done, rs));
-                    OCRS_HIP(hipStreamWaitEvent(st, done, 0));
+                    if (rs == st || ws.stream.may_park_waits()) OCRS_HIP(hipStreamWaitEvent(st, done, 0));
+                    else rec_done = done;
                 }
+                if (rec_done) ws.host_wait(rec_done);
             }
             if (ran_persistent) {
             } else if (fused) {
diff --git a/ocrs_amd/csrc/model.hpp b/ocrs_amd/csrc/model.hpp
--- a/ocrs_amd/csrc/model.hpp
+++ b/ocrs_amd/csrc/model.hpp
@@ -112,7 +112,8 @@
                                float** d_logp = nullptr, float* d_maxlp = nullptr, OpRange* range = nullptr) const;
     float* run_prefix_ragged(Workspace& ws, hipStream_t exec, const std::vector<PackedGroup>& groups,
                              const PackedPlan& plan, int h, int ts, StageTimers* timers, int* feat_c,
-                             const std::function<void()>& before_launch = nullptr, const OpRange* range = nullptr) const;
+                             const std::function<void()>& before_launch = nullptr, const OpRange* range = nullptr,
+                             hipEvent_t* stack_done = nullptr) const;
 };
 
 }
diff --git a/ocrs_amd/csrc/stream_plan.hpp b/ocrs_amd/csrc/stream_plan.hpp
--- /dev/null
+++ b/ocrs_amd/csrc/stream_plan.hpp
@@ -0,0 +1,56 @@
+#pragma once
+#include <mutex>
+#include <vector>
+
+namespace ocrs {
+
+class LanePlan {
+  public:
+    enum { kMinBudget = 3, kMaxBudget = 16, kDefaultBudget = 4, kPrivate = -1 };
+    static bool valid_budget(long b) { return b == 0 || (b >= kMinBudget && b <= kMaxBudget); }
+
+    explicit LanePlan(int budget = kDefaultBudget) { (void)set_budget(budget); }
+
+    bool set_budget(int budget) {
+        std::lock_guard<std::mutex> g(mu_);
+        if (!valid_budget(budget)) return false;
+        if (budget == budget_) return true;
+        if (outstanding_ > 0) return false;
+        budget_ = budget;
+        load_.assign(budget ? budget - 2 : 0, 0);
+        next_ = 0;
+        return true;
+    }
+    int budget() const { std::lock_guard<std::mutex> g(mu_); return budget_; }
+    int light_lanes() const { std::lock_guard<std::mutex> g(mu_); return (int)load_.size(); }
+    int outstanding() const { std::lock_guard<std::mutex> g(mu_); return outstanding_; }
+    int load(int lane) const { std::lock_guard<std::mutex> g(mu_); return lane >= 0 && lane < (int)load_.size() ? load_[lane] : 0; }
+
+    int acquire(int avoid = kPrivate) {
+        std::lock_guard<std::mutex> g(mu_);
+        outstanding_++;
+        const int n = (int)load_.size();
+        if (n == 0) return kPrivate;
+        int best = -1;
+        for (int i = 0; i < n; i++) {
+            const int lane = (next_ + i) % n;
+            if (lane == avoid && n > 1) continue;
+            if (best < 0 || load_[lane] < load_[best]) best = lane;
+        }
+        load_[best]++;
+        next_ = (best + 1) % n;
+        return best;
+    }
+    void release(int lane) {
+        std::lock_guard<std::mutex> g(mu_);
+        outstanding_--;
+        if (lane >= 0 && lane < (int)load_.size()) load_[lane]--;
+    }
+
+  private:
+    mutable std::mutex mu_;
+    int budget_ = -1, outstanding_ = 0, next_ = 0;
+    std::vector<int> load_;
+};
+
+}
```

Result: faster. 276.5, median of 6 (+1.6%).
